# mcgill-cpslab/all-pairs-similarity

Measured on AMD Instinct MI355X. Metric: scored candidate pairs/sec + achieved HBM GB/s, N=1M d=100k nnz=100, 1/2/4/8 GPU, higher is better.
Workload: dtype u16+f32

## Files before the change

all-pairs-similarity_amd/csrc/apss_hip.hip:

```cpp
#include <hip/hip_runtime.h>

#include <algorithm>
#include <cmath>
#include <cstdio>
#include <cstdlib>
#include <cstring>
#include <new>
#include <string>
#include <vector>

#include "../../include/apss.h"
#include "apss_kernels.hpp"
#include "apss_head.hpp"
#include "apss_even.hpp"
#include "apss_topk.hpp"

using namespace apss;

namespace {

thread_local std::string g_create_error;

template <class T>
struct DevBuf {
  T *p = nullptr;
  size_t cap = 0;
};

struct DebugCfg {
  bool build_lds = false;
  bool build_atomic = false;
  bool build_stream = false;
  bool build_runs = false;
  int run_range = 0;
  int run_lanes = 0;
  int run_sub = -1;
  bool build_trace = false;
  bool chunk8 = false;
  bool shard_exact = false;
  bool diag = false;
  bool force_general = false;
  bool exact_accum = false;
  bool big_u5 = false;
  int cx_tile = 0;
  int window = 0;
  int chunks = 0;
  int tiles_per_launch = 0;
  bool no_tail = false;
  bool no_acc8 = false;
  int flat_group = -1;
  int pad_lds = 0;
  bool longpf = false;
  bool even_wide = false;
  bool no_even = false;
  int seg_align = 0;
  bool bank_order = false;
  int fold_w = 0;
  bool no_sym = false;
  int mix = 0;
  bool no_chain = false;
  bool no_append = false;
  bool no_bucket = false;
  int bucket_range = 0;
  int res_cap = 0;
  bool head_bf16 = false;
  int merge = -1;
  bool no_merge_prune = false;
  int merge_u = 0;
  int merge_single = 0;
};

DebugCfg parse_debug_env() {
  DebugCfg d;
  const char *e = getenv("APSS_DEBUG");
  if (!e) return d;
  std::string str(e);
  size_t pos = 0;
  while (pos <= str.size()) {
    const size_t end = std::min(str.find(',', pos), str.size());
    const std::string tok = str.substr(pos, end - pos);
    pos = end + 1;
    const size_t eq = tok.find('=');
    const std::string key = tok.substr(0, eq);
    const int val = eq == std::string::npos ? 1 : atoi(tok.c_str() + eq + 1);
    if (key == "build_lds") d.build_lds = val != 0;
    else if (key == "build_atomic") d.build_atomic = val != 0;
    else if (key == "build_stream") d.build_stream = val != 0;
    else if (key == "build_runs") d.build_runs = val != 0;
    else if (key == "run_range") d.run_range = val;
    else if (key == "run_lanes") d.run_lanes = val;
    else if (key == "run_sub") d.run_sub = val;
    else if (key == "build_trace") d.build_trace = val != 0;
    else if (key == "chunk8") d.chunk8 = val != 0;
    else if (key == "shard_exact") d.shard_exact = val != 0;
    else if (key == "diag") d.diag = val != 0;
    else if (key == "force_general") d.force_general = val != 0;
    else if (key == "exact_accum") d.exact_accum = val != 0;
    else if (key == "big_u5") d.big_u5 = val != 0;
    else if (key == "cx_tile") d.cx_tile = val;
    else if (key == "window") d.window = val;
    else if (key == "chunks") d.chunks = val;
    else if (key == "tiles_per_launch") d.tiles_per_launch = val;
    else if (key == "no_tail") d.no_tail = val != 0;
    else if (key == "no_acc8") d.no_acc8 = val != 0;
    else if (key == "no_even") d.no_even = val != 0;
    else if (key == "even_wide") d.even_wide = val != 0;
    else if (key == "longpf") d.longpf = val != 0;
    else if (key == "pad_lds") d.pad_lds = (int)val;
    else if (key == "flat_group") d.flat_group = (int)val;
    else if (key == "seg_align") d.seg_align = val;
    else if (key == "bank_order") d.bank_order = val != 0;
    else if (key == "fold_w") d.fold_w = val;
    else if (key == "mix") d.mix = val;
    else if (key == "no_sym") d.no_sym = val != 0;
    else if (key == "no_chain") d.no_chain = val != 0;
    else if (key == "no_append") d.no_append = val != 0;
    else if (key == "head_bf16") d.head_bf16 = val != 0;
    else if (key == "res_cap") d.res_cap = val;
    else if (key == "no_bucket") d.no_bucket = val != 0;
    else if (key == "bucket_range") d.bucket_range = val;
    else if (key == "merge") d.merge = (int)val;
    else if (key == "merge_u") d.merge_u = (int)val;
    else if (key == "no_merge_prune") d.no_merge_prune = val != 0;
    else if (key == "merge_single") d.merge_single = (int)val;
    else if (key == "relayout_fail") {}
    else if (!key.empty()) fprintf(stderr, "[apss] unknown APSS_DEBUG token '%s' ignored\n", key.c_str());
  }
  return d;
}

}

struct apss_handle {
  apss_config cfg{};
  DebugCfg dbgcfg;
  int dev = 0;
  hipStream_t own_stream = nullptr;
  hipStream_t stream = nullptr;
  hipEvent_t ev0 = nullptr, ev1 = nullptr;
  std::string err;
  bool sharded = false;
  bool nonneg = true;
  bool q_nonneg = true;
  bool no_acc8 = false;
  uint32_t downgrades = 0;
  int64_t store_max_nnz = 0, q_max_nnz = 0;
  float store_max_norm2 = 0.f, q_max_norm2 = 0.f;
  int64_t store_nonempty = 0;
  int64_t last_batch_nonempty = 0;
  int32_t cb = 16384;
  bool stored_rows = false;

  int64_t n_rows = 0, nnz = 0;
  int64_t idx_rows = 0;
  DevBuf<int64_t> rowptr, ext;
  DevBuf<int32_t> idx;
  DevBuf<uint32_t> erow;
  DevBuf<float> val, sub;
  struct IndexSet {
    int32_t cb = 0;
    int32_t align = 0;
    bool coarse = false;
    int64_t n_tiles = 0, post_used = 0;
    DevBuf<uint2> seg;
    DevBuf<Posting> post;
    DevBuf<uint32_t> post_c;
    DevBuf<int64_t> base, total;
    DevBuf<uint32_t> scan_part;
    DevBuf<uint32_t> maxlen;
    uint32_t max_seg = 0;
    uint32_t long_segs = 0;
    DevBuf<unsigned long long> chunkw;
    double round_chunks = 0.0;
    std::vector<int64_t> h_base;
    double build_ms = 0;
    int64_t built_rows = 0;
  };
  IndexSet ex, cx;
  bool use_coarse = false;
  int64_t n_tiles = 0;
  int64_t ex_built_rows = 0;
  DevBuf<float> tile_min, tile_min_c;
  DevBuf<int64_t> q_rowptr, q_ext;
  DevBuf<int32_t> q_idx;
  DevBuf<float> q_val, q_sub;
  DevBuf<int64_t> s_keep, s_cnt, s_rowdst, s_nnzdst, in_rowptr, in_ext;
  DevBuf<int64_t> scan_tmp;
  DevBuf<int32_t> in_idx;
  DevBuf<float> s_inv, s_sub, in_val;
  DevBuf<double> in_val64;
  DevBuf<unsigned long long> bk_cnt;
  DevBuf<int64_t> bk_base;
  DevBuf<int32_t> bk_idx;
  DevBuf<uint32_t> bk_erow;
  DevBuf<float> bk_val;
  DevBuf<uint32_t> run_cut;
  DevBuf<uint2> run_ent;
  DevBuf<uint2> app_seg;
  DevBuf<char> app_post;
  DevBuf<int32_t> vq_first, vrow_q;
  DevBuf<int64_t> vrow_ptr, vrow_np, vrow_first;
  DevBuf<int32_t> res_q, res_c, fin_q, fin_c;
  DevBuf<float> res_s, fin_s;
  DevBuf<int32_t> res2_q, res2_c;
  DevBuf<float> res2_s, q_prenorm;
  const int32_t *out_q = nullptr, *out_c = nullptr;
  const float *out_s = nullptr;
  int64_t n_res = -1;
  const int64_t *res_q_ext = nullptr;
  const int64_t *last_q_rowptr = nullptr;
  const int32_t *last_q_idx = nullptr;
  const float *last_q_val = nullptr;
  int64_t last_nq = 0;
  DevBuf<unsigned long long> counters, dbg, chain_ctr;
  DevBuf<unsigned int> flagword;
  char *pin = nullptr;
  DevBuf<char> pack;
  const int64_t *up_rowptr = nullptr, *up_ext = nullptr;
  const int32_t *up_idx = nullptr;
  int32_t head_k = 0;
  bool head_fixed = false;
  int32_t head_fold_w = 128;
  int32_t head_exact = 128;
  int32_t head_fold_user = 0;
  bool merge_off = false;
  bool head_longseg = false;
  int32_t head_part = 0, head_parts = 1;
  int64_t head_eval_rows = 0;
  bool head_blocked = false;
  std::vector<int32_t> head_terms;
  DevBuf<int32_t> head_pos;
  struct TailView {
    DevBuf<int64_t> rowptr;
    DevBuf<int32_t> idx;
    DevBuf<float> val;
    DevBuf<uint32_t> erow;
    int64_t rows = 0, nnz = 0, max_nnz = 0, nonempty = 0, last_nonempty = 0;
  };
  TailView tv, qtv;
  DevBuf<int64_t> tv_cnt, tv_off;
  DevBuf<unsigned int> tv_sum;
  DevBuf<uint16_t> W, q_W;
  bool head_i8 = false;
  float head_s = 0.f;
  DevBuf<unsigned int> head_ovf;
  DevBuf<uint32_t> df;
  DevBuf<unsigned long long> dedup_tab, head_ctr;
  DevBuf<int32_t> uq_q, uq_c;
  DevBuf<float> uq_s;
  int64_t head_nonempty = 0, last_batch_head_nonempty = 0;
  double head_sample_frac = 0.0;
  hipEvent_t ev2 = nullptr, ev3 = nullptr;
  int32_t top_k = 0;
  TopkWork topk;
  apss_topk_info tk{};
  apss_stats st{};
  size_t bytes_reserved = 0;
};

namespace {

#define HIPCHK(h, expr)                                                                              \
  do {                                                                                               \
    hipError_t e_ = (expr);                                                                          \
    if (e_ != hipSuccess) {                                                                          \
      (h)->err = std::string(#expr) + ": " + hipGetErrorString(e_);                                  \
      return e_ == hipErrorOutOfMemory ? APSS_E_NOMEM : APSS_E_DEVICE;                               \
    }                                                                                                \
  } while (0)

#define APSS_TRY(expr)          \
  do {                          \
    int32_t rc_ = (expr);       \
    if (rc_ != APSS_OK) return rc_; \
  } while (0)

int32_t fail(apss_handle *h, int32_t rc, const std::string &msg) {
  h->err = msg;
  return rc;
}

template <class T>
int32_t ensure(apss_handle *h, DevBuf<T> &b, size_t n, size_t keep = 0, bool exact = false) {
  if (n <= b.cap && b.p) return APSS_OK;
  size_t ncap = exact ? n : std::max(n, b.cap + b.cap / 2);
  ncap = std::max<size_t>(ncap, 64);
  T *np = nullptr;
  HIPCHK(h, hipMalloc((void **)&np, ncap * sizeof(T)));
  if (keep && b.p) HIPCHK(h, hipMemcpyAsync(np, b.p, keep * sizeof(T), hipMemcpyDeviceToDevice, h->stream));
  if (b.p) {
    HIPCHK(h, hipStreamSynchronize(h->stream));
    HIPCHK(h, hipFree(b.p));
    h->bytes_reserved -= b.cap * sizeof(T);
  }
  b.p = np;
  b.cap = ncap;
  h->bytes_reserved += ncap * sizeof(T);
  return APSS_OK;
}

template <class T>
void release(DevBuf<T> &b) {
  if (b.p) (void)hipFree(b.p);
  b.p = nullptr;
  b.cap = 0;
}

int32_t enter(apss_handle *h) {
  if (!h) return APSS_E_INVALID;
  hipError_t e = hipSetDevice(h->dev);
  if (e != hipSuccess) return fail(h, APSS_E_DEVICE, std::string("hipSetDevice: ") + hipGetErrorString(e));
  return APSS_OK;
}

inline int64_t ceil_div(int64_t a, int64_t b) { return (a + b - 1) / b; }
constexpr size_t kPinBytes = 256 << 10;
constexpr size_t kPinScalars = 1024;

int32_t scan_i64(apss_handle *h, const int64_t *in, int64_t *out, int64_t n) {
  if (n <= 4 * kScanBlock) {
    hipLaunchKernelGGL(k_scan_i64, dim3(1), dim3(1024), 0, h->stream, in, out, n);
    HIPCHK(h, hipGetLastError());
    return APSS_OK;
  }
  const int64_t nb = ceil_div(n, kScanBlock);
  APSS_TRY(ensure(h, h->scan_tmp, (size_t)(2 * nb + 1)));
  int64_t *sums = h->scan_tmp.p, *offs = h->scan_tmp.p + nb;
  hipLaunchKernelGGL(k_scan_sums, dim3((unsigned)nb), dim3(1024), 0, h->stream, in, sums, n);
  hipLaunchKernelGGL(k_scan_i64, dim3(1), dim3(1024), 0, h->stream, (const int64_t *)sums, offs, nb);
  hipLaunchKernelGGL(k_scan_apply, dim3((unsigned)nb), dim3(1024), 0, h->stream, in, (const int64_t *)offs, out, n, nb);
  HIPCHK(h, hipGetLastError());
  return APSS_OK;
}

int32_t head_setup_rendering(apss_handle *h);
int32_t head_fit_scale(apss_handle *h, double norm2, unsigned char *W, int64_t packed_bytes);
inline void head_pack_rendering(const apss_handle *h, HeadPackArgs &p);

int32_t ingest(apss_handle *h, int64_t n, int64_t nnz, const int64_t *d_rowptr, const int32_t *d_idx,
               const float *d_val, const int64_t *d_ext, bool to_store, int64_t *n_out, int64_t *nnz_out) {
  *n_out = 0;
  *nnz_out = 0;
  if (n == 0) return APSS_OK;
  const uint32_t in_flags = h->stored_rows ? h->cfg.flags & ~(APSS_FLAG_VALUE_PRUNE | APSS_FLAG_ADMISSION | APSS_FLAG_NORMALIZE) : h->cfg.flags;
  const bool transform = h->sharded || (in_flags & (APSS_FLAG_VALUE_PRUNE | APSS_FLAG_ADMISSION | APSS_FLAG_NORMALIZE));
  APSS_TRY(ensure(h, h->s_keep, (size_t)n + 1));
  APSS_TRY(ensure(h, h->s_cnt, (size_t)n + 1));
  APSS_TRY(ensure(h, h->s_inv, (size_t)n));
  APSS_TRY(ensure(h, h->s_sub, (size_t)n));
  APSS_TRY(ensure(h, h->flagword, 4));
  HIPCHK(h, hipMemsetAsync(h->flagword.p, 0, 4 * sizeof(unsigned int), h->stream));

  IngestArgs a{};
  a.n = n;
  a.nnz = nnz;
  a.rowptr = d_rowptr;
  a.idx = d_idx;
  a.val = d_val;
  a.dim = h->cfg.dim;
  a.term_lo = h->cfg.term_lo;
  a.term_hi = h->cfg.term_hi;
  a.flags = in_flags;
  a.theta = (float)h->cfg.theta;
  a.index_threshold = (float)h->cfg.index_threshold;
  a.row_keep = h->s_keep.p;
  a.row_cnt = h->s_cnt.p;
  a.row_inv = h->s_inv.p;
  a.row_sub = h->s_sub.p;
  a.flags_out = h->flagword.p;
  const bool shard_head = h->sharded && h->head_k > 0;
  a.head_pos = shard_head ? h->head_pos.p : nullptr;
  const int threads = 256;
  const int64_t blocks = ceil_div(n * kGroup, threads);
  hipLaunchKernelGGL(k_ingest_count<kGroup>, dim3((unsigned)std::min<int64_t>(blocks, 4096)), dim3(threads), 0, h->stream, a);
  HIPCHK(h, hipGetLastError());

  int64_t dst_row0 = to_store ? h->n_rows : 0, dst_nnz0 = to_store ? h->nnz : 0;
  int64_t kept_rows = n, kept_nnz = nnz;
  unsigned int flags_stack[4] = {0, 0, 0, 0};
  unsigned int *flags_host = h->pin ? reinterpret_cast<unsigned int *>(h->pin + kPinBytes) : flags_stack;
  if (transform) {
    APSS_TRY(ensure(h, h->s_rowdst, (size_t)n + 1));
    APSS_TRY(ensure(h, h->s_nnzdst, (size_t)n + 1));
    APSS_TRY(scan_i64(h, (const int64_t *)h->s_keep.p, h->s_rowdst.p, n));
    APSS_TRY(scan_i64(h, (const int64_t *)h->s_cnt.p, h->s_nnzdst.p, n));
    HIPCHK(h, hipGetLastError());
    HIPCHK(h, hipMemcpyAsync(&kept_rows, h->s_rowdst.p + n, sizeof(int64_t), hipMemcpyDeviceToHost, h->stream));
    HIPCHK(h, hipMemcpyAsync(&kept_nnz, h->s_nnzdst.p + n, sizeof(int64_t), hipMemcpyDeviceToHost, h->stream));
  }
  HIPCHK(h, hipMemcpyAsync(flags_host, h->flagword.p, 4 * sizeof(unsigned int), hipMemcpyDeviceToHost, h->stream));
  HIPCHK(h, hipStreamSynchronize(h->stream));
  if (flags_host[0] & 1u)
    return fail(h, APSS_E_INVALID, "malformed vector: indices must be strictly increasing and in [0, dim) "
                                   "(SparseVector.scala:75; vectorDim mismatch is the require of CommonUtils.scala:99)");
  if (flags_host[0] & 2u) return fail(h, APSS_E_INVALID, "non-finite value in a vector");
  if (to_store) h->nonneg = h->nonneg && !(flags_host[0] & 4u);
  else h->q_nonneg = !(flags_host[0] & 4u);
  float norm2;
  std::memcpy(&norm2, &flags_host[2], sizeof(float));
  if (to_store) {
    h->store_max_nnz = std::max<int64_t>(h->store_max_nnz, flags_host[1]);
    h->store_max_norm2 = std::max(h->store_max_norm2, norm2);
    h->store_nonempty += flags_host[3];
    h->last_batch_nonempty = flags_host[3];
  } else {
    h->q_max_nnz = flags_host[1];
    h->q_max_norm2 = norm2;
  }

  DevBuf<int64_t> &o_rowptr = to_store ? h->rowptr : h->q_rowptr;
  DevBuf<int64_t> &o_ext = to_store ? h->ext : h->q_ext;
  DevBuf<int32_t> &o_idx = to_store ? h->idx : h->q_idx;
  DevBuf<float> &o_val = to_store ? h->val : h->q_val;
  DevBuf<float> &o_sub = to_store ? h->sub : h->q_sub;
  APSS_TRY(ensure(h, o_rowptr, (size_t)(dst_row0 + kept_rows + 1), (size_t)(to_store ? dst_row0 + 1 : 0)));
  APSS_TRY(ensure(h, o_ext, (size_t)(dst_row0 + kept_rows), (size_t)dst_row0));
  APSS_TRY(ensure(h, o_idx, (size_t)(dst_nnz0 + kept_nnz), (size_t)dst_nnz0));
  APSS_TRY(ensure(h, o_val, (size_t)(dst_nnz0 + kept_nnz), (size_t)dst_nnz0));
  if (to_store) APSS_TRY(ensure(h, h->erow, (size_t)(dst_nnz0 + kept_nnz), (size_t)dst_nnz0));
  if (h->sharded) APSS_TRY(ensure(h, o_sub, (size_t)(dst_row0 + kept_rows), (size_t)dst_row0));
  if (dst_row0 == 0) HIPCHK(h, hipMemsetAsync(o_rowptr.p, 0, sizeof(int64_t), h->stream));

  IngestWriteArgs w{};
  w.in = a;
  w.dst_row0 = dst_row0;
  w.dst_nnz0 = dst_nnz0;
  w.o_rowptr = o_rowptr.p;
  w.o_idx = o_idx.p;
  w.o_val = o_val.p;
  w.o_ext = o_ext.p;
  w.o_sub = h->sharded ? o_sub.p : nullptr;
  w.o_erow = to_store ? h->erow.p : nullptr;
  w.ext = d_ext;
  if (transform) {
    w.row_dst = h->s_rowdst.p;
    w.nnz_dst = h->s_nnzdst.p;
  } else {
    w.row_dst = nullptr;
    w.nnz_dst = d_rowptr;
  }
  hipLaunchKernelGGL(k_ingest_write, dim3((unsigned)blocks), dim3(threads), 0, h->stream, w);
  HIPCHK(h, hipGetLastError());
  if (shard_head) {
    const int64_t kh = h->head_k;
    DevBuf<uint16_t> &o_W = to_store ? h->W : h->q_W;
    const int64_t rows_end = dst_row0 + kept_rows;
    const int64_t w_pad = to_store ? ceil_div(rows_end, kHeadQBlock) * kHeadQBlock + kHeadCTile : ceil_div(rows_end, kHeadCTile) * kHeadCTile;
    APSS_TRY(ensure(h, o_W, (size_t)(w_pad * kh), (size_t)(ceil_div(dst_row0, kHeadCTile) * kHeadCTile * kh)));
    APSS_TRY(ensure(h, h->head_ctr, 4));
    HIPCHK(h, hipMemsetAsync(h->head_ctr.p, 0, 4 * sizeof(unsigned long long), h->stream));
    if (to_store && dst_row0 == 0) APSS_TRY(head_setup_rendering(h));
    APSS_TRY(head_fit_scale(h, to_store ? (double)h->store_max_norm2 : std::max((double)h->store_max_norm2, (double)h->q_max_norm2),
                            reinterpret_cast<unsigned char *>(h->W.p), ceil_div(to_store ? dst_row0 : h->n_rows, kHeadCTile) * kHeadCTile * kh));
    HeadPackArgs p{};
    head_pack_rendering(h, p);
    p.rowptr = d_rowptr;
    p.idx = d_idx;
    p.val = d_val;
    p.row0 = 0;
    p.row1 = n;
    p.head_pos = h->head_pos.p;
    p.kh = (int32_t)kh;
    p.W = o_W.p;
    p.w_row0 = dst_row0;
    p.w_pad = w_pad;
    p.ratio_t = nullptr;
    p.head_nonempty = reinterpret_cast<unsigned int *>(h->head_ctr.p);
    p.row_inv = (in_flags & APSS_FLAG_NORMALIZE) ? h->s_inv.p : nullptr;
    p.prune_above = (in_flags & APSS_FLAG_VALUE_PRUNE) ? (float)h->cfg.index_threshold : -INFINITY;
    p.fold_from = h->head_exact;
    p.part = h->head_part;
    p.n_parts = h->head_parts;
    hipLaunchKernelGGL(k_head_pack, dim3((unsigned)(ceil_div(w_pad, 8) - dst_row0 / 8)), dim3(512), 0, h->stream, p);
    HIPCHK(h, hipGetLastError());
    if (to_store) {
      unsigned int nz = 0;
      HIPCHK(h, hipMemcpyAsync(&nz, h->head_ctr.p, sizeof(nz), hipMemcpyDeviceToHost, h->stream));
      HIPCHK(h, hipStreamSynchronize(h->stream));
      if (dst_row0 == 0) h->head_nonempty = 0;
      h->head_nonempty += nz;
      h->last_batch_head_nonempty = nz;
    }
  }
  *n_out = kept_rows;
  *nnz_out = kept_nnz;
  return APSS_OK;
}

void fill_build_args(apss_handle *h, apss_handle::IndexSet &ix, BuildArgs &b, bool scaled) {
  b.rowptr = h->head_k ? h->tv.rowptr.p : h->rowptr.p;
  b.idx = h->head_k ? h->tv.idx.p : h->idx.p;
  b.val = h->head_k ? h->tv.val.p : h->val.p;
  b.cb = (int32_t)ix.cb;
  b.dim = h->cfg.dim;
  b.tile_seg = ix.seg.p;
  b.seg_stride = (int64_t)h->cfg.dim;
  b.coarse = ix.coarse ? 1 : 0;
  b.seg_align = ix.align;
  b.erow = h->head_k ? h->tv.erow.p : h->erow.p;
  b.row_scale = scaled && ix.coarse ? h->sub.p : nullptr;
  b.coarse_shift = ix.coarse && ix.cb <= 32768 ? 1 : 0;
  b.coarse_wide = ix.coarse && ix.cb > 65536 ? 1 : 0;
  b.tile_post_base = ix.base.p;
  b.post = ix.post.p;
  b.post_c = ix.post_c.p;
  b.term_lo = h->cfg.term_lo;
  b.term_hi = h->cfg.term_hi;
}

int32_t launch_tile_scan(apss_handle *h, apss_handle::IndexSet &ix, int64_t tile0, int64_t n, uint32_t keep_len, unsigned long long *chunk_w,
                         uint32_t count_long) {
  const int32_t n_blk = (int32_t)ceil_div(h->cfg.dim, kScanBlock);
  APSS_TRY(ensure(h, ix.scan_part, (size_t)(n * n_blk)));
  const dim3 grid((unsigned)(n * n_blk));
  hipLaunchKernelGGL(k_tile_scan_part, grid, dim3(1024), 0, h->stream, (const uint2 *)ix.seg.p, (int64_t)h->cfg.dim, h->cfg.dim, tile0, n_blk,
                     (uint32_t)ix.align, ix.scan_part.p, ix.maxlen.p, chunk_w, count_long);
  hipLaunchKernelGGL(k_tile_scan_place, grid, dim3(1024), 0, h->stream, ix.seg.p, (int64_t)h->cfg.dim, h->cfg.dim, tile0, n_blk, (uint32_t)ix.align,
                     keep_len, (const uint32_t *)ix.scan_part.p, ix.total.p);
  HIPCHK(h, hipGetLastError());
  return APSS_OK;
}

int32_t append_tile(apss_handle *h, apss_handle::IndexSet &ix, int64_t tile, int64_t row0, int64_t row1) {
  const int64_t stride = (int64_t)h->cfg.dim;
  const bool scaled = h->sharded || h->head_k > 0;
  const size_t elt = ix.coarse ? sizeof(uint32_t) : sizeof(Posting);
  const int64_t base = ix.h_base[(size_t)tile], old_total = ix.h_base[(size_t)tile + 1] - base;
  uint2 *sg = ix.seg.p + tile * stride;
  APSS_TRY(ensure(h, h->app_seg, (size_t)stride));
  APSS_TRY(ensure(h, h->app_post, (size_t)std::max<int64_t>(old_total, 1) * elt));
  HIPCHK(h, hipEventRecord(h->ev0, h->stream));
  HIPCHK(h, hipMemcpyAsync(h->app_seg.p, sg, (size_t)stride * sizeof(uint2), hipMemcpyDeviceToDevice, h->stream));
  if (old_total > 0)
    HIPCHK(h, hipMemcpyAsync(h->app_post.p, ix.coarse ? (const void *)(ix.post_c.p + base) : (const void *)(ix.post.p + base),
                             (size_t)old_total * elt, hipMemcpyDeviceToDevice, h->stream));
  BuildArgs b{};
  fill_build_args(h, ix, b, scaled);
  b.row0 = row0;
  b.row1 = row1;
  const int threads = 256;
  const int64_t blocks = ceil_div((row1 - row0) * kWave, threads);
  hipLaunchKernelGGL(k_tile_hist, dim3((unsigned)blocks), dim3(threads), 0, h->stream, b);
  APSS_TRY(launch_tile_scan(h, ix, tile, 1, 0u, nullptr, 0u));
  HIPCHK(h, hipGetLastError());
  int64_t new_total = 0;
  uint32_t seg_stats[2] = {0, 0};
  HIPCHK(h, hipMemcpyAsync(&new_total, ix.total.p + tile, sizeof(int64_t), hipMemcpyDeviceToHost, h->stream));
  HIPCHK(h, hipMemcpyAsync(seg_stats, ix.maxlen.p, sizeof(seg_stats), hipMemcpyDeviceToHost, h->stream));
  HIPCHK(h, hipStreamSynchronize(h->stream));
  ix.max_seg = seg_stats[0];
  ix.h_base[(size_t)tile + 1] = base + new_total;
  ix.post_used = base + new_total;
  if (ix.coarse) APSS_TRY(ensure(h, ix.post_c, (size_t)ix.post_used + 64, (size_t)base));
  else APSS_TRY(ensure(h, ix.post, (size_t)ix.post_used + 64, (size_t)base));
  if (ix.coarse)
    HIPCHK(h, hipMemsetAsync(ix.post_c.p + base, 0, (size_t)(new_total + 64) * sizeof(uint32_t), h->stream));
  HIPCHK(h, hipMemcpyAsync(ix.base.p + tile + 1, ix.h_base.data() + tile + 1, sizeof(int64_t), hipMemcpyHostToDevice, h->stream));
  ShiftArgs sa{};
  sa.seg_old = h->app_seg.p;
  sa.seg_new = sg;
  sa.old_c = ix.coarse ? reinterpret_cast<const uint32_t *>(h->app_post.p) : nullptr;
  sa.old_x = ix.coarse ? nullptr : reinterpret_cast<const Posting *>(h->app_post.p);
  sa.new_c = ix.coarse ? ix.post_c.p + base : nullptr;
  sa.new_x = ix.coarse ? nullptr : ix.post.p + base;
  sa.dim = h->cfg.dim;
  hipLaunchKernelGGL(k_tile_shift, dim3((unsigned)ceil_div(stride * kGroup, 256)), dim3(256), 0, h->stream, sa);
  fill_build_args(h, ix, b, scaled);
  b.row0 = row0;
  b.row1 = row1;
  hipLaunchKernelGGL(k_tile_scatter, dim3((unsigned)blocks), dim3(threads), 0, h->stream, b);
  if (scaled) {
    DevBuf<float> &tmin = ix.coarse ? h->tile_min_c : h->tile_min;
    hipLaunchKernelGGL(k_tile_min_sub, dim3(1), dim3(1024), 0, h->stream, (const float *)h->sub.p, h->idx_rows, (int32_t)ix.cb, tmin.p, tile);
  }
  HIPCHK(h, hipGetLastError());
  HIPCHK(h, hipEventRecord(h->ev1, h->stream));
  HIPCHK(h, hipEventSynchronize(h->ev1));
  float ms = 0.f;
  HIPCHK(h, hipEventElapsedTime(&ms, h->ev0, h->ev1));
  ix.build_ms = ms;
  return APSS_OK;
}

constexpr double kRunMinMeanRow = 20.0;
constexpr int kRunSub = 256;
template <int SCATTER>
void launch_tile_runs(int lanes, dim3 grid, size_t lds, hipStream_t stream, const BuildArgs &b, int64_t tile0, int32_t n_ranges) {
  if (lanes == 4) hipLaunchKernelGGL((k_tile_runs<SCATTER, 4>), grid, dim3(1024), lds, stream, b, tile0, n_ranges);
  else if (lanes == 8) hipLaunchKernelGGL((k_tile_runs<SCATTER, 8>), grid, dim3(1024), lds, stream, b, tile0, n_ranges);
  else if (lanes == 16) hipLaunchKernelGGL((k_tile_runs<SCATTER, 16>), grid, dim3(1024), lds, stream, b, tile0, n_ranges);
  else hipLaunchKernelGGL((k_tile_runs<SCATTER, 32>), grid, dim3(1024), lds, stream, b, tile0, n_ranges);
}

int32_t build_tiles(apss_handle *h, apss_handle::IndexSet &ix, int64_t row0) {
  const int64_t cb = ix.cb;
  int64_t tile0 = row0 / cb;
  const int64_t n_tiles = ceil_div(h->idx_rows, cb);
  const int64_t stride = (int64_t)h->cfg.dim;
  double appended_ms = 0.0;
  if (row0 % cb != 0 && ix.built_rows == row0 && ix.n_tiles == tile0 + 1 && (int64_t)ix.h_base.size() == tile0 + 2 &&
      !h->dbgcfg.no_append && !h->dbgcfg.bank_order) {
    DevBuf<float> &tmin_a = ix.coarse ? h->tile_min_c : h->tile_min;
    if (h->sharded || h->head_k > 0) APSS_TRY(ensure(h, tmin_a, (size_t)n_tiles, (size_t)tile0 + 1));
    APSS_TRY(ensure(h, ix.total, (size_t)n_tiles, (size_t)tile0 + 1));
    APSS_TRY(append_tile(h, ix, tile0, row0, std::min<int64_t>(h->idx_rows, (tile0 + 1) * cb)));
    appended_ms = ix.build_ms;
    ++tile0;
    row0 = tile0 * cb;
    if (h->idx_rows <= row0) {
      ix.built_rows = h->idx_rows;
      return APSS_OK;
    }
  }
  ix.n_tiles = n_tiles;
  ix.built_rows = h->idx_rows;
  if (n_tiles == tile0) return APSS_OK;
  APSS_TRY(ensure(h, ix.seg, (size_t)(n_tiles * stride), (size_t)(tile0 * stride)));
  APSS_TRY(ensure(h, ix.base, (size_t)n_tiles + 1, (size_t)tile0 + 1));
  APSS_TRY(ensure(h, ix.total, (size_t)n_tiles, 0));
  APSS_TRY(ensure(h, ix.maxlen, 2));
  APSS_TRY(ensure(h, ix.chunkw, 1));
  if (tile0 == 0) {
    HIPCHK(h, hipMemsetAsync(ix.maxlen.p, 0, 2 * sizeof(uint32_t), h->stream));
    HIPCHK(h, hipMemsetAsync(ix.chunkw.p, 0, sizeof(unsigned long long), h->stream));
  }
  DevBuf<float> &tmin = ix.coarse ? h->tile_min_c : h->tile_min;
  const bool scaled = h->sharded || h->head_k > 0;
  if (scaled) APSS_TRY(ensure(h, tmin, (size_t)n_tiles, (size_t)tile0));
  if (ix.h_base.empty()) ix.h_base.push_back(0);
  ix.h_base.resize((size_t)tile0 + 1);
  const int64_t r0 = tile0 * cb;
  int32_t n_ranges = (int32_t)ceil_div(h->cfg.dim, kBuildRange);
  const int64_t build_nnz = h->head_k ? h->tv.nnz : h->nnz;
  int32_t bucket_rt = h->dbgcfg.bucket_range > 0 ? h->dbgcfg.bucket_range : 8192;
  while (ceil_div(h->cfg.dim, bucket_rt) > kBucketMaxRanges && bucket_rt < kBuildRange) bucket_rt *= 2;
  const bool bucket_build = n_ranges > kBuildMaxRanges && ceil_div(h->cfg.dim, bucket_rt) <= kBucketMaxRanges && !h->dbgcfg.build_atomic &&
                            !h->dbgcfg.no_bucket && tile0 == 0 && n_tiles * n_ranges >= 48 && build_nnz > 0 && build_nnz <= (1LL << 32) &&
                            n_tiles * (int64_t)kBucketSlices < (1LL << 31);
  if (bucket_build) n_ranges = (int32_t)ceil_div(h->cfg.dim, bucket_rt);
  const bool lds_build = bucket_build || (n_ranges <= kBuildMaxRanges && !h->dbgcfg.build_atomic &&
                                          ((n_tiles - tile0) * n_ranges >= 48 || h->dbgcfg.build_lds));
  if (!lds_build)
    HIPCHK(h, hipMemsetAsync(ix.seg.p + tile0 * stride, 0, (size_t)((n_tiles - tile0) * stride) * sizeof(uint2), h->stream));
  const double mean_row = h->idx_rows > 0 ? (double)build_nnz / (double)h->idx_rows : 0.0;
  int32_t run_rt = h->dbgcfg.run_range > 0 ? std::min(h->dbgcfg.run_range, kBuildRange) : kRunRange;
  const int64_t t_lo = h->cfg.term_lo, t_hi = h->cfg.term_hi;
  const int64_t run_active = std::max<int64_t>(1, ceil_div(t_hi, run_rt) - t_lo / run_rt);
  const double mean_run = mean_row / (double)run_active;
  const bool run_build = lds_build && !bucket_build && !h->dbgcfg.build_stream && std::max<int64_t>(h->store_max_nnz, 1) * cb < (1LL << 31) &&
                         ceil_div(h->cfg.dim, run_rt) <= 64 &&
                         (h->dbgcfg.build_runs || (n_ranges >= 2 && mean_row >= kRunMinMeanRow));
  if (run_build) n_ranges = (int32_t)ceil_div(h->cfg.dim, run_rt);
  BuildArgs b{};
  fill_build_args(h, ix, b, scaled);
  b.row0 = r0;
  b.row1 = h->idx_rows;
  int32_t run_sub = h->dbgcfg.run_sub >= 0 ? h->dbgcfg.run_sub : kRunSub;
  if (run_sub < 64 || run_sub > kPlaceMaxTerms || (run_sub & (run_sub - 1)) || run_rt % run_sub || !ix.coarse || build_nnz > (int64_t)6e8 || build_nnz <= 0)
    run_sub = 0;
  const int32_t n_sub = run_sub ? (int32_t)ceil_div(h->cfg.dim, run_sub) : 0;
  const int64_t n_bk = (n_tiles - tile0) * n_sub;
  const double run_want = run_sub ? mean_run * 0.5 : mean_run;
  int run_lanes = h->dbgcfg.run_lanes;
  if (run_lanes != 4 && run_lanes != 8 && run_lanes != 16 && run_lanes != 32)
    run_lanes = run_want <= 4.0 ? 4 : (run_want <= 8.0 ? 8 : (run_want <= 16.0 ? 16 : 32));
  if (h->dbgcfg.build_trace)
    fprintf(stderr, "[apss] build %s tiles [%lld, %lld): %s, %d ranges of %d terms, %d lanes per row (mean run %.2f)\n", ix.coarse ? "coarse" : "exact",
            (long long)tile0, (long long)n_tiles, bucket_build ? "bucketed" : (run_build ? "runs" : (lds_build ? "stream" : "atomic")), (int)n_ranges,
            run_build ? run_rt : (bucket_build ? bucket_rt : kBuildRange), run_build ? run_lanes : 0, mean_run);
  if (h->dbgcfg.build_trace && run_build) fprintf(stderr, "[apss]   scatter through sub-ranges of %d terms\n", (int)run_sub);
  if (run_build) {
    APSS_TRY(ensure(h, h->run_cut, (size_t)((h->idx_rows - r0) * (n_ranges + 1))));
    b.range_terms = run_rt;
    b.run_cut = h->run_cut.p;
    if (run_sub) {
      APSS_TRY(ensure(h, h->bk_cnt, (size_t)n_bk + 2));
      APSS_TRY(ensure(h, h->bk_base, (size_t)n_bk + 2));
      APSS_TRY(ensure(h, h->run_ent, (size_t)build_nnz));
      int sh = 0;
      while ((1 << sh) < run_sub) ++sh;
      b.sub_shift = sh;
      b.n_sub = n_sub;
      b.sub_cnt = h->bk_cnt.p;
      b.sub_base = h->bk_base.p;
      b.o_ent = h->run_ent.p;
    }
  }
  const int threads = 256;
  const int64_t blocks = ceil_div((h->idx_rows - r0) * kWave, threads);
  HIPCHK(h, hipEventRecord(h->ev0, h->stream));
  int64_t group_tiles = n_tiles;
  BucketArgs bk{};
  if (bucket_build) {
    const int64_t per_tile = std::max<int64_t>(1, build_nnz / n_tiles);
    group_tiles = std::max<int64_t>(1, std::min<int64_t>(n_tiles, (int64_t)6e8 / per_tile));
    std::vector<int64_t> grp_e;
    {
      std::vector<int64_t> at;
      for (int64_t g0 = 0; g0 < n_tiles; g0 += group_tiles) at.push_back(std::min<int64_t>(h->idx_rows, g0 * cb));
      at.push_back(h->idx_rows);
      grp_e.resize(at.size());
      for (size_t i = 0; i < at.size(); ++i)
        HIPCHK(h, hipMemcpyAsync(&grp_e[i], b.rowptr + at[i], sizeof(int64_t), hipMemcpyDeviceToHost, h->stream));
      HIPCHK(h, hipStreamSynchronize(h->stream));
    }
    int64_t max_e = 1;
    for (size_t i = 0; i + 1 < grp_e.size(); ++i) max_e = std::max(max_e, grp_e[i + 1] - grp_e[i]);
    const int64_t nb = group_tiles * n_ranges;
    APSS_TRY(ensure(h, h->bk_cnt, (size_t)(2 * nb + 2)));
    APSS_TRY(ensure(h, h->bk_base, (size_t)nb + 2));
    APSS_TRY(ensure(h, h->bk_idx, (size_t)max_e));
    APSS_TRY(ensure(h, h->bk_erow, (size_t)max_e));
    APSS_TRY(ensure(h, h->bk_val, (size_t)max_e));
    bk.rowptr = b.rowptr;
    bk.idx = b.idx;
    bk.val = b.val;
    bk.erow = b.erow;
    bk.row1 = h->idx_rows;
    bk.cb = (int32_t)cb;
    bk.n_ranges = n_ranges;
    bk.range_terms = bucket_rt;
    bk.bucket_cnt = h->bk_cnt.p;
    bk.bucket_cur = h->bk_cnt.p + nb + 1;
    bk.bucket_base = h->bk_base.p;
    bk.o_idx = h->bk_idx.p;
    bk.o_erow = h->bk_erow.p;
    bk.o_val = h->bk_val.p;
    HIPCHK(h, hipEventRecord(h->ev0, h->stream));
  }
  auto bucket_group = [&](int64_t g0, int64_t gt) -> int32_t {
    const int64_t nbg = gt * n_ranges;
    HIPCHK(h, hipMemsetAsync(h->bk_cnt.p, 0, (size_t)(2 * (group_tiles * n_ranges) + 2) * sizeof(unsigned long long), h->stream));
    bk.tile0 = g0;
    const dim3 bgrid((unsigned)(gt * kBucketSlices));
    hipLaunchKernelGGL(k_bucket_pass<false>, bgrid, dim3(1024), 0, h->stream, bk);
    APSS_TRY(scan_i64(h, reinterpret_cast<const int64_t *>(h->bk_cnt.p), h->bk_base.p, nbg));
    hipLaunchKernelGGL(k_bucket_pass<true>, bgrid, dim3(1024), 0, h->stream, bk);
    HIPCHK(h, hipGetLastError());
    return APSS_OK;
  };
  if (bucket_build) {
    b.idx = h->bk_idx.p;
    b.erow = h->bk_erow.p;
    b.val = h->bk_val.p;
    b.ent_base = h->bk_base.p;
    b.range_terms = bucket_rt;
    for (int64_t g0 = 0; g0 < n_tiles; g0 += group_tiles) {
      const int64_t gt = std::min<int64_t>(group_tiles, n_tiles - g0);
      APSS_TRY(bucket_group(g0, gt));
      hipLaunchKernelGGL(k_tile_hist_lds, dim3((unsigned)(gt * n_ranges)), dim3(1024), 0, h->stream, b, g0, n_ranges);
    }
    HIPCHK(h, hipGetLastError());
  }
  const dim3 lds_grid((unsigned)((n_tiles - tile0) * n_ranges));
  const size_t run_lds = (size_t)run_rt * sizeof(uint32_t);
  if (bucket_build) {}
  else if (run_build) {
    hipLaunchKernelGGL(k_row_cuts, dim3((unsigned)ceil_div((h->idx_rows - r0) * kGroup, threads)), dim3(threads), 0, h->stream, b, n_ranges,
                       h->run_cut.p);
    launch_tile_runs<kRunHist>(run_lanes, lds_grid, run_lds, h->stream, b, tile0, n_ranges);
    if (run_sub) {
      APSS_TRY(scan_i64(h, reinterpret_cast<const int64_t *>(h->bk_cnt.p), h->bk_base.p, n_bk));
      launch_tile_runs<kRunPartition>(run_lanes, lds_grid, run_lds, h->stream, b, tile0, n_ranges);
    }
  } else if (lds_build) hipLaunchKernelGGL(k_tile_hist_lds, lds_grid, dim3(1024), 0, h->stream, b, tile0, n_ranges);
  else hipLaunchKernelGGL(k_tile_hist, dim3((unsigned)blocks), dim3(threads), 0, h->stream, b);
  APSS_TRY(launch_tile_scan(h, ix, tile0, n_tiles - tile0, lds_build ? 1u : 0u, tile0 == 0 ? ix.chunkw.p : nullptr, 1u));
  HIPCHK(h, hipGetLastError());
  std::vector<int64_t> tot((size_t)(n_tiles - tile0));
  HIPCHK(h, hipMemcpyAsync(tot.data(), ix.total.p + tile0, tot.size() * sizeof(int64_t), hipMemcpyDeviceToHost, h->stream));
  uint32_t seg_stats[2] = {0, 0};
  unsigned long long chunk_w = 0;
  HIPCHK(h, hipMemcpyAsync(seg_stats, ix.maxlen.p, sizeof(seg_stats), hipMemcpyDeviceToHost, h->stream));
  HIPCHK(h, hipMemcpyAsync(&chunk_w, ix.chunkw.p, sizeof(chunk_w), hipMemcpyDeviceToHost, h->stream));
  HIPCHK(h, hipStreamSynchronize(h->stream));
  ix.max_seg = seg_stats[0];
  ix.long_segs = seg_stats[1];
  if (tile0 == 0 && h->idx_rows > 0) ix.round_chunks = (double)chunk_w / (double)h->idx_rows;
  for (size_t i = 0; i < tot.size(); ++i) ix.h_base.push_back(ix.h_base.back() + tot[i]);
  HIPCHK(h, hipMemcpyAsync(ix.base.p + tile0, ix.h_base.data() + tile0, (size_t)(n_tiles - tile0 + 1) * sizeof(int64_t),
                           hipMemcpyHostToDevice, h->stream));
  ix.post_used = ix.h_base.back();
  if (ix.coarse) APSS_TRY(ensure(h, ix.post_c, (size_t)ix.post_used + 64, (size_t)ix.h_base[(size_t)tile0]));
  else APSS_TRY(ensure(h, ix.post, (size_t)ix.post_used + 64, (size_t)ix.h_base[(size_t)tile0]));
  if (ix.coarse)
    HIPCHK(h, hipMemsetAsync(ix.post_c.p + ix.h_base[(size_t)tile0], 0,
                             (size_t)(ix.post_used - ix.h_base[(size_t)tile0] + 64) * sizeof(uint32_t), h->stream));
  b.tile_post_base = ix.base.p;
  b.post = ix.post.p;
  b.post_c = ix.post_c.p;
  if (bucket_build) {
    for (int64_t g0 = 0; g0 < n_tiles; g0 += group_tiles) {
      const int64_t gt = std::min<int64_t>(group_tiles, n_tiles - g0);
      if (group_tiles < n_tiles) APSS_TRY(bucket_group(g0, gt));
      hipLaunchKernelGGL(k_tile_scatter_lds, dim3((unsigned)(gt * n_ranges)), dim3(1024), 0, h->stream, b, g0, n_ranges);
    }
  } else if (run_build && run_sub) {
    hipLaunchKernelGGL(k_tile_place_sub, dim3((unsigned)n_bk), dim3(kPlaceBlock), 0, h->stream, b, tile0);
  } else if (run_build) launch_tile_runs<kRunScatter>(run_lanes, lds_grid, run_lds, h->stream, b, tile0, n_ranges);
  else if (lds_build) hipLaunchKernelGGL(k_tile_scatter_lds, lds_grid, dim3(1024), 0, h->stream, b, tile0, n_ranges);
  else hipLaunchKernelGGL(k_tile_scatter, dim3((unsigned)blocks), dim3(threads), 0, h->stream, b);
  if (ix.coarse && ix.cb <= 32768 && h->dbgcfg.bank_order)
    hipLaunchKernelGGL(k_seg_bank_order, dim3((unsigned)ceil_div((n_tiles - tile0) * stride * kWave, 256)), dim3(256), 0, h->stream,
                       (const uint2 *)ix.seg.p, stride, (const int64_t *)ix.base.p, ix.post_c.p, tile0, n_tiles, h->cfg.dim);
  if (scaled)
    hipLaunchKernelGGL(k_tile_min_sub, dim3((unsigned)(n_tiles - tile0)), dim3(1024), 0, h->stream,
                       (const float *)h->sub.p, h->idx_rows, (int32_t)cb, tmin.p, tile0);
  HIPCHK(h, hipGetLastError());
  HIPCHK(h, hipEventRecord(h->ev1, h->stream));
  HIPCHK(h, hipEventSynchronize(h->ev1));
  float ms = 0.f;
  HIPCHK(h, hipEventElapsedTime(&ms, h->ev0, h->ev1));
  ix.build_ms = ms + appended_ms;
  return APSS_OK;
}

int32_t ensure_exact_index(apss_handle *h) {
  if (h->ex_built_rows < h->idx_rows || h->ex.n_tiles == 0) {
    APSS_TRY(build_tiles(h, h->ex, std::min(h->ex_built_rows, h->idx_rows)));
    h->ex_built_rows = h->idx_rows;
    h->st.build_ms += h->ex.build_ms;
  }
  return APSS_OK;
}

double acc8_scale(double bound, double shared, double theta) {
  for (int k = 7; k >= 5; --k) {
    const double S = std::ldexp(1.0, k);
    if (bound * 1.0005 * S < 255.0 - shared && std::floor(theta * S * (1.0 - 1.0 / 2048 - 1e-6)) - 2 >= 12.0) return S;
  }
  return 0.0;
}

constexpr int64_t kTailMaxRows = 1024;
constexpr int64_t kTailMaxBatch = 64;
constexpr int64_t kTailMaxPairs = 1 << 22;
constexpr int32_t kHeadMaxTerms = kHeadBlock * (1 + kHeadMaxFold);
inline int32_t head_width(int32_t n_terms, int32_t fold_w, int32_t exact = kHeadBlock, bool i8 = false) {
  return n_terms <= 64 ? (i8 ? 128 : 64) : (n_terms <= 128 ? 128 : (n_terms <= 256 ? 256 : exact + fold_w));
}
inline int32_t head_column(int32_t i, int32_t fold_w, int32_t exact = kHeadBlock) { return i < exact ? i : exact + (i - exact) % fold_w; }
constexpr int64_t kHeadMinRows = 16384;
constexpr double kHeadSparseRate = 8.0e11;
constexpr double kHeadDenseCost[4] = {1.5e-13, 1.9e-13, 3.1e-13, 3.1e-13};
constexpr double kHeadDenseCostI8[4] = {1.2e-13, 1.2e-13, 1.75e-13, 1.75e-13};
constexpr double kHeadFoldMaxRowTerms = 96.0;
constexpr double kHeadSurvivorCost = 2.5e-9;

inline bool head_allowed(const apss_handle *h) {
  return h->use_coarse && (!h->sharded || h->head_fixed) && (h->cfg.head_terms >= 0 || h->head_fixed) && h->cfg.theta > 0.0 &&
         !h->head_blocked && h->nonneg;
}

inline bool head_wants_i8(const apss_handle *h) {
  return !h->dbgcfg.head_bf16 && !(h->dbgcfg.fold_w == 128 || h->dbgcfg.fold_w == 256);
}
int32_t head_setup_rendering(apss_handle *h) {
  h->head_i8 = h->head_k > 0 && h->head_k <= kHeadBlock && head_wants_i8(h);
  h->head_s = 0.f;
  APSS_TRY(ensure(h, h->head_ovf, 4));
  HIPCHK(h, hipMemsetAsync(h->head_ovf.p, 0, 4 * sizeof(unsigned int), h->stream));
  return APSS_OK;
}
int32_t head_fit_scale(apss_handle *h, double norm2, unsigned char *W, int64_t packed_bytes) {
  if (!h->head_i8) return APSS_OK;
  const double need = 127.0 / (std::sqrt(std::max(norm2, 1e-30)) * 1.0005);
  if (h->head_s > 0.f && need >= (double)h->head_s) return APSS_OK;
  if (h->head_s > 0.f && packed_bytes > 0) {
    const double target = need / 1.25;
    const uint32_t den = 65535u;
    const uint32_t num = (uint32_t)std::min<double>(den, std::ceil(target / (double)h->head_s * den));
    hipLaunchKernelGGL(k_head_rescale, dim3((unsigned)std::min<int64_t>(8192, ceil_div(packed_bytes, 16 * 256))), dim3(256), 0, h->stream, W,
                       packed_bytes / 16 * 16, num, den);
    HIPCHK(h, hipGetLastError());
    h->head_s = (float)target;
  } else {
    h->head_s = (float)need;
  }
  return APSS_OK;
}
inline void head_pack_rendering(const apss_handle *h, HeadPackArgs &p) {
  p.i8_scale = h->head_i8 ? h->head_s : 0.f;
  p.overflow = h->head_ovf.p;
}

int32_t build_tail_view(apss_handle *h, apss_handle::TailView &v, const int64_t *rowptr, const int32_t *idx, const float *val,
                        int64_t row0, int64_t row1, int64_t dst_row0, bool with_erow) {
  const int64_t n = row1 - row0;
  if (dst_row0 == 0) v.rows = v.nnz = v.max_nnz = v.nonempty = 0;
  v.last_nonempty = 0;
  APSS_TRY(ensure(h, v.rowptr, (size_t)(dst_row0 + n + 1), (size_t)(dst_row0 ? dst_row0 + 1 : 0)));
  if (dst_row0 == 0) HIPCHK(h, hipMemsetAsync(v.rowptr.p, 0, sizeof(int64_t), h->stream));
  if (n <= 0) return APSS_OK;
  APSS_TRY(ensure(h, h->tv_cnt, (size_t)n + 1));
  APSS_TRY(ensure(h, h->tv_off, (size_t)n + 1));
  APSS_TRY(ensure(h, h->tv_sum, 2));
  HIPCHK(h, hipMemsetAsync(h->tv_sum.p, 0, 2 * sizeof(unsigned int), h->stream));
  TailViewArgs a{};
  a.rowptr = rowptr;
  a.idx = idx;
  a.val = val;
  a.row0 = row0;
  a.row1 = row1;
  a.head_pos = h->head_pos.p;
  a.cnt = h->tv_cnt.p;
  a.summary = h->tv_sum.p;
  const unsigned blocks = (unsigned)ceil_div(n * kGroup, 256);
  hipLaunchKernelGGL(k_tailv_count, dim3(blocks), dim3(256), 0, h->stream, a);
  HIPCHK(h, hipGetLastError());
  APSS_TRY(scan_i64(h, (const int64_t *)h->tv_cnt.p, h->tv_off.p, n));
  int64_t total = 0;
  unsigned int sum[2] = {0, 0};
  HIPCHK(h, hipMemcpyAsync(&total, h->tv_off.p + n, sizeof(int64_t), hipMemcpyDeviceToHost, h->stream));
  HIPCHK(h, hipMemcpyAsync(sum, h->tv_sum.p, sizeof(sum), hipMemcpyDeviceToHost, h->stream));
  HIPCHK(h, hipStreamSynchronize(h->stream));
  const int64_t nnz0 = v.nnz;
  APSS_TRY(ensure(h, v.idx, (size_t)std::max<int64_t>(nnz0 + total, 1), (size_t)nnz0));
  APSS_TRY(ensure(h, v.val, (size_t)std::max<int64_t>(nnz0 + total, 1), (size_t)nnz0));
  if (with_erow) APSS_TRY(ensure(h, v.erow, (size_t)std::max<int64_t>(nnz0 + total, 1), (size_t)nnz0));
  a.off = h->tv_off.p;
  a.dst_row0 = dst_row0;
  a.dst_nnz0 = nnz0;
  a.o_rowptr = v.rowptr.p;
  a.o_idx = v.idx.p;
  a.o_val = v.val.p;
  a.o_erow = with_erow ? v.erow.p : nullptr;
  hipLaunchKernelGGL(k_tailv_write, dim3(blocks), dim3(256), 0, h->stream, a);
  HIPCHK(h, hipGetLastError());
  v.rows = dst_row0 + n;
  v.nnz = nnz0 + total;
  v.max_nnz = std::max<int64_t>(v.max_nnz, sum[0]);
  v.nonempty += sum[1];
  v.last_nonempty = sum[1];
  return APSS_OK;
}

int32_t head_pack_store(apss_handle *h, int64_t row0) {
  const int64_t kh = h->head_k;
  const int64_t rows_pad = ceil_div(h->idx_rows, kHeadQBlock) * kHeadQBlock + kHeadCTile;
  APSS_TRY(ensure(h, h->W, (size_t)(rows_pad * kh), (size_t)(ceil_div(row0, kHeadCTile) * kHeadCTile * kh)));
  APSS_TRY(ensure(h, h->sub, (size_t)h->idx_rows, (size_t)row0));
  APSS_TRY(ensure(h, h->head_ctr, 4));
  HIPCHK(h, hipMemsetAsync(h->head_ctr.p, 0, 4 * sizeof(unsigned long long), h->stream));
  if (row0 == 0) APSS_TRY(head_setup_rendering(h));
  APSS_TRY(head_fit_scale(h, (double)h->store_max_norm2, reinterpret_cast<unsigned char *>(h->W.p), ceil_div(row0, kHeadCTile) * kHeadCTile * kh));
  {
    HeadPackArgs a{};
    head_pack_rendering(h, a);
    a.rowptr = h->rowptr.p;
    a.idx = h->idx.p;
    a.val = h->val.p;
    a.row0 = row0;
    a.row1 = h->idx_rows;
    a.head_pos = h->head_pos.p;
    a.kh = (int32_t)kh;
    a.W = h->W.p;
    a.w_row0 = row0;
    a.w_pad = rows_pad;
    a.ratio_t = h->sub.p;
    a.head_nonempty = reinterpret_cast<unsigned int *>(h->head_ctr.p);
    a.row_inv = nullptr;
    a.prune_above = -INFINITY;
    a.fold_from = h->head_exact;
    hipLaunchKernelGGL(k_head_pack, dim3((unsigned)(ceil_div(rows_pad, 8) - row0 / 8)), dim3(512), 0, h->stream, a);
  }
  HIPCHK(h, hipGetLastError());
  unsigned int nz = 0;
  HIPCHK(h, hipMemcpyAsync(&nz, h->head_ctr.p, sizeof(nz), hipMemcpyDeviceToHost, h->stream));
  HIPCHK(h, hipStreamSynchronize(h->stream));
  if (row0 == 0) h->head_nonempty = 0;
  h->head_nonempty += nz;
  h->last_batch_head_nonempty = nz;
  return APSS_OK;
}

int32_t run_head(apss_handle *h, const ProbeArgs &a, int64_t nq, int64_t q_slot_base, const uint16_t *Wq, int64_t wq_rows,
                 float thr, double bound, int64_t n_cand);

int32_t head_sample_selectivity(apss_handle *h, double *frac) {
  *frac = 0.0;
  const int64_t kh = h->head_k;
  const int64_t S = std::min<int64_t>(h->idx_rows, 8192), Q = std::min<int64_t>(S, 512);
  const int64_t rows_pad = ceil_div(h->idx_rows, kHeadQBlock) * kHeadQBlock + kHeadCTile;
  APSS_TRY(ensure(h, h->W, (size_t)(rows_pad * kh), 0));
  APSS_TRY(ensure(h, h->sub, (size_t)h->idx_rows, 0));
  APSS_TRY(ensure(h, h->head_ctr, 4));
  APSS_TRY(ensure(h, h->counters, kCtrCount));
  HIPCHK(h, hipMemsetAsync(h->head_ctr.p, 0, 4 * sizeof(unsigned long long), h->stream));
  APSS_TRY(head_setup_rendering(h));
  APSS_TRY(head_fit_scale(h, (double)h->store_max_norm2, nullptr, 0));
  HeadPackArgs p{};
  head_pack_rendering(h, p);
  p.rowptr = h->rowptr.p;
  p.idx = h->idx.p;
  p.val = h->val.p;
  p.row0 = 0;
  p.row1 = S;
  p.head_pos = h->head_pos.p;
  p.kh = (int32_t)kh;
  p.W = h->W.p;
  p.w_row0 = 0;
  p.w_pad = ceil_div(S, kHeadQBlock) * kHeadQBlock;
  p.ratio_t = h->sub.p;
  p.head_nonempty = nullptr;
  p.row_inv = nullptr;
  p.prune_above = -INFINITY;
  p.fold_from = h->head_exact;
  hipLaunchKernelGGL(k_head_pack, dim3((unsigned)ceil_div(p.w_pad, 8)), dim3(512), 0, h->stream, p);
  HIPCHK(h, hipGetLastError());
  constexpr size_t kSampleCap = 1 << 20;
  APSS_TRY(ensure(h, h->res_q, kSampleCap));
  APSS_TRY(ensure(h, h->res_c, kSampleCap));
  APSS_TRY(ensure(h, h->res_s, kSampleCap));
  ProbeArgs a{};
  a.q_ext = h->ext.p;
  a.res_q = h->res_q.p;
  a.res_c = h->res_c.p;
  a.res_s = h->res_s.p;
  a.res_cap = kSampleCap;
  a.counters = h->head_ctr.p + 2;
  const double bound = (double)h->store_max_norm2 * 1.0001 + 1e-6;
  APSS_TRY(run_head(h, a, Q, -1, h->W.p, p.w_pad, (float)(h->cfg.theta - 0.0080 * bound - 1e-5), bound, S));
  unsigned long long c[4];
  HIPCHK(h, hipMemcpyAsync(c, h->head_ctr.p, sizeof(c), hipMemcpyDeviceToHost, h->stream));
  HIPCHK(h, hipStreamSynchronize(h->stream));
  const double pairs = (double)Q * (double)S - (double)Q;
  unsigned long long n_true = 0;
  if (c[2] > 0 && c[2] <= kSampleCap) {
    APSS_TRY(ensure(h, h->fin_q, (size_t)c[2]));
    APSS_TRY(ensure(h, h->fin_c, (size_t)c[2]));
    APSS_TRY(ensure(h, h->fin_s, (size_t)c[2]));
    HIPCHK(h, hipMemsetAsync(h->head_ctr.p, 0, sizeof(unsigned long long), h->stream));
    RescoreArgs r{};
    r.n_pairs = (int64_t)c[2];
    r.q_row = h->res_q.p;
    r.c_slot = h->res_c.p;
    r.q_rowptr = h->rowptr.p;
    r.q_idx = h->idx.p;
    r.q_val = h->val.p;
    r.c_rowptr = h->rowptr.p;
    r.c_idx = h->idx.p;
    r.c_val = h->val.p;
    r.theta = (float)h->cfg.theta;
    r.out_q = h->fin_q.p;
    r.out_c = h->fin_c.p;
    r.out_s = h->fin_s.p;
    r.out_count = h->head_ctr.p;
    hipLaunchKernelGGL(k_rescore, dim3((unsigned)std::max<int64_t>(1, ceil_div(r.n_pairs, (int64_t)kRescorePairs * kRescoreTrips))), dim3(kRescoreBlock), 0, h->stream, r);
    HIPCHK(h, hipGetLastError());
    HIPCHK(h, hipMemcpyAsync(&n_true, h->head_ctr.p, sizeof(n_true), hipMemcpyDeviceToHost, h->stream));
    HIPCHK(h, hipStreamSynchronize(h->stream));
  }
  *frac = pairs > 0 ? (double)(c[2] - std::min(n_true, c[2])) / pairs : 0.0;
  return APSS_OK;
}

int32_t choose_head(apss_handle *h, bool *changed) {
  *changed = false;
  const int64_t n = h->n_rows;
  const int32_t dim = h->cfg.dim;
  h->head_eval_rows = n;
  const int64_t stride = std::max<int64_t>(1, n / 65536);
  const int64_t sampled = ceil_div(n, stride);
  APSS_TRY(ensure(h, h->df, (size_t)dim));
  HIPCHK(h, hipMemsetAsync(h->df.p, 0, (size_t)dim * sizeof(uint32_t), h->stream));
  hipLaunchKernelGGL(k_df_sample, dim3((unsigned)ceil_div(sampled * kWave, 256)), dim3(256), 0, h->stream,
                     (const int64_t *)h->rowptr.p, (const int32_t *)h->idx.p, n, stride, h->df.p);
  HIPCHK(h, hipGetLastError());
  std::vector<uint32_t> df((size_t)dim);
  HIPCHK(h, hipMemcpyAsync(df.data(), h->df.p, (size_t)dim * sizeof(uint32_t), hipMemcpyDeviceToHost, h->stream));
  HIPCHK(h, hipStreamSynchronize(h->stream));
  std::vector<int32_t> order((size_t)dim);
  for (int32_t t = 0; t < dim; ++t) order[(size_t)t] = t;
  const size_t top = (size_t)std::min<int32_t>(dim, kHeadMaxTerms);
  const auto more_frequent = [&](int32_t x, int32_t y) { return df[(size_t)x] != df[(size_t)y] ? df[(size_t)x] > df[(size_t)y] : x < y; };
  bool hopeless = false;
  if (h->cfg.head_terms == 0) {
    double s2_all = 0.0, f_max = 0.0;
    for (int32_t t = 0; t < dim; ++t) {
      const double f = (double)df[(size_t)t] / (double)sampled;
      s2_all += f * f;
      f_max = std::max(f_max, f);
    }
    const double *cost = head_wants_i8(h) ? kHeadDenseCostI8 : kHeadDenseCost;
    const double terms_of[4] = {64.0, 128.0, 256.0, (double)top};
    hopeless = true;
    for (int ki = 0; ki < 4; ++ki)
      if (std::min(s2_all, terms_of[ki] * f_max * f_max) / kHeadSparseRate >= 1.5 * 0.5 * cost[ki]) hopeless = false;
  }
  if (!hopeless) {
    std::nth_element(order.begin(), order.begin() + (ptrdiff_t)top - 1, order.end(), more_frequent);
    std::sort(order.begin(), order.begin() + (ptrdiff_t)top, more_frequent);
  }
  int32_t k = 0;
  double best_gain = 0.0;
  double gain256 = 0.0;
  if (h->cfg.head_terms > 0) {
    k = std::min(h->cfg.head_terms <= 256 ? head_width(h->cfg.head_terms, 0) : h->cfg.head_terms, kHeadMaxTerms);
  } else if (n >= kHeadMinRows && !hopeless) {
    double best = 0.0, s2 = 0.0;
    size_t i = 0;
    int ki = 0;
    double m_fold = 0.0;
    for (int32_t kk : {64, 128, 256, 512, 1024, 2048, 4096, 8192, 16384, 32768}) {
      if (kk > kHeadMaxTerms || (size_t)kk > top + 255) break;
      for (; i < std::min<size_t>(top, (size_t)kk); ++i) {
        const double f = (double)df[(size_t)order[i]] / (double)sampled;
        s2 += f * f;
        if (i >= (size_t)h->head_exact) m_fold += f;
      }
      if (m_fold > kHeadFoldMaxRowTerms) break;
      const double save = s2 / kHeadSparseRate, cost = 0.5 * (head_wants_i8(h) ? kHeadDenseCostI8 : kHeadDenseCost)[std::min(ki++, 3)];
      if (save >= 1.5 * cost && kk == kHeadBlock) gain256 = save - cost;
      if (save >= 1.5 * cost && save - cost > best) {
        best = save - cost;
        k = kk;
      }
    }
    best_gain = best;
  }
  if (std::min(k, kHeadBlock) > dim) k = 0;
  std::vector<int32_t> terms;
  for (size_t i = 0; i < std::min<size_t>(top, (size_t)k); ++i)
    if (df[(size_t)order[i]] > 0) terms.push_back(order[i]);
  const int32_t old_k = h->head_k;
  const std::vector<int32_t> old_terms = h->head_terms;
  auto upload_columns = [&]() -> int32_t {
    std::vector<int32_t> pos((size_t)dim, -1);
    for (size_t i = 0; i < h->head_terms.size(); ++i) pos[(size_t)h->head_terms[i]] = head_column((int32_t)i, h->head_fold_w, h->head_exact);
    APSS_TRY(ensure(h, h->head_pos, (size_t)dim));
    HIPCHK(h, hipMemcpyAsync(h->head_pos.p, pos.data(), (size_t)dim * sizeof(int32_t), hipMemcpyHostToDevice, h->stream));
    HIPCHK(h, hipStreamSynchronize(h->stream));
    return APSS_OK;
  };
  for (;;) {
    k = terms.empty() ? 0 : head_width((int32_t)terms.size(), h->head_fold_w, h->head_exact, head_wants_i8(h));
    const bool differs = k != old_k || terms != old_terms;
    h->head_k = k;
    h->head_terms = terms;
    if (k && differs) APSS_TRY(upload_columns());
    if (!(k && differs && h->cfg.head_terms == 0)) break;
    double frac = 0.0;
    APSS_TRY(head_sample_selectivity(h, &frac));
    h->head_sample_frac = frac;
    if (frac * kHeadSurvivorCost <= 0.5 * best_gain) break;
    if (terms.size() > (size_t)kHeadBlock && gain256 > 0.0) {
      terms.resize((size_t)kHeadBlock);
      best_gain = gain256;
      continue;
    }
    h->head_k = 0;
    h->head_terms.clear();
    break;
  }
  *changed = h->head_k != old_k || h->head_terms != old_terms;
  return APSS_OK;
}

int32_t build_index(apss_handle *h, int64_t row0) {
  h->st.build_ms = 0;
  row0 = std::min(row0, h->idx_rows);
  h->idx_rows = h->n_rows;
  if (head_allowed(h)) {
    if (!h->head_fixed && h->n_rows >= std::max<int64_t>(h->cfg.head_terms > 0 ? 1 : kHeadMinRows, 2 * h->head_eval_rows)) {
      bool changed = false;
      APSS_TRY(choose_head(h, &changed));
      if (changed) {
        row0 = 0;
        h->cx.n_tiles = 0;
        h->ex_built_rows = 0;
      }
    }
    if (h->head_k) {
      h->cx.cb = std::min(h->cx.cb, 65536);
      if (!h->sharded) APSS_TRY(head_pack_store(h, row0));
      const int64_t tv0 = row0 == h->tv.rows ? row0 : 0;
      APSS_TRY(build_tail_view(h, h->tv, h->rowptr.p, h->idx.p, h->val.p, tv0, h->idx_rows, tv0, true));
    }
  } else if (h->head_k && h->sharded) {
    return fail(h, APSS_E_UNSUPPORTED, "a term shard with a dense-head block needs non-negative weights (apss_set_head_terms)");
  } else if (h->head_k) {
    h->downgrades |= APSS_DOWNGRADE_HEAD;
    h->head_k = 0;
    h->head_terms.clear();
    row0 = 0;
    h->cx.n_tiles = 0;
    h->ex_built_rows = 0;
  }
  if (h->use_coarse) {
    if (h->cx.n_tiles == 0 && h->cfg.tile_rows == 0 && !h->dbgcfg.cx_tile && h->idx_rows > 0) {
      const double seg32 = 32768.0 * ((double)h->nnz / (double)h->n_rows) / (double)h->cfg.dim;
      h->cx.cb = seg32 < 16.0 && !h->sharded && !h->head_k ? 65536 : 32768;
      if (h->cx.cb == 65536 && seg32 < 8.0 && h->nonneg && !h->dbgcfg.no_acc8 && !h->no_acc8 && h->store_max_nnz <= 512 &&
          acc8_scale((double)h->store_max_norm2 * 1.0001 + 1e-6, (double)h->store_max_nnz, h->cfg.theta) > 0)
        h->cx.cb = 131072;
      if ((h->sharded || h->head_k) && !(h->head_k && h->head_longseg) && !h->dbgcfg.no_acc8 && !h->no_acc8 &&
          acc8_scale((double)h->store_max_norm2 * 1.0001 + 1e-6, (double)h->store_max_nnz, h->cfg.theta) > 0)
        h->cx.cb = 65536;
    }
    APSS_TRY(build_tiles(h, h->cx, row0));
    h->st.build_ms += h->cx.build_ms;
    if (h->head_k && h->cfg.tile_rows == 0 && !h->dbgcfg.cx_tile) {
      if (h->cx.cb > 32768 && h->cx.max_seg > (uint32_t)kLongLenW) {
        h->head_longseg = true;
        h->cx.cb = 32768;
        h->cx.n_tiles = 0;
        APSS_TRY(build_tiles(h, h->cx, 0));
        h->st.build_ms += h->cx.build_ms;
      } else if (h->cx.cb <= 32768 && h->head_longseg && row0 == 0 && 2 * h->cx.max_seg <= (uint32_t)kLongLenW) {
        h->head_longseg = false;
      }
    }
    h->ex_built_rows = std::min(h->ex_built_rows, row0 / h->ex.cb * h->ex.cb);
  } else {
    h->ex_built_rows = std::min(h->ex_built_rows, row0);
    APSS_TRY(ensure_exact_index(h));
  }
  h->n_tiles = ceil_div(h->idx_rows, h->ex.cb);
  return APSS_OK;
}

template <int MODE, bool FX, int BLOCK = kProbeBlock>
int32_t launch_probe(apss_handle *h, const ProbeArgs &a, size_t lds) {
  auto kern = k_probe<MODE, BLOCK, FX>;
  HIPCHK(h, hipFuncSetAttribute(reinterpret_cast<const void *>(kern), hipFuncAttributeMaxDynamicSharedMemorySize, (int)lds));
  hipLaunchKernelGGL(kern, dim3((unsigned)((int64_t)a.n_tiles * a.n_chunks)), dim3(BLOCK), lds, h->stream, a);
  HIPCHK(h, hipGetLastError());
  return APSS_OK;
}
inline int gen_block(int mode, int cb) { return mode == 2 && cb <= 8192 ? 512 : kProbeBlock; }

#define APSS_CX_VARIANTS(X)                          \
  X(512, 5, false, 16, false, false, false, false)   \
  X(512, 4, false, 16, false, false, false, false)   \
  X(512, 3, false, 16, false, false, false, false)   \
  X(512, 2, false, 16, false, false, false, false)   \
  X(512, 5, true, 16, false, false, false, false)    \
  X(512, 4, true, 16, false, false, false, false)    \
  X(512, 3, true, 16, false, false, false, false)    \
  X(512, 2, true, 16, false, false, false, false)    \
  X(512, 5, true, 16, false, false, false, true)     \
  X(512, 4, true, 16, false, false, false, true)     \
  X(512, 3, true, 16, false, false, false, true)     \
  X(512, 2, true, 16, false, false, false, true)     \
  X(512, 5, false, 16, false, false, false, true)    \
  X(512, 4, false, 16, false, false, false, true)    \
  X(512, 3, false, 16, false, false, false, true)    \
  X(512, 2, false, 16, false, false, false, true)    \
  X(512, 5, true, 16, false, false, true, false)     \
  X(512, 5, false, 16, false, false, true, false)    \
  X(512, 5, true, 16, true, false, true, false)      \
  X(512, 4, false, 8, false, false, false, false)    \
  X(512, 5, false, 16, true, false, false, false)    \
  X(512, 5, false, 16, false, true, false, false)    \
  X(512, 5, true, 16, false, true, false, false)     \
  X(512, 5, false, 16, true, true, false, false)     \
  X(1024, 5, false, 16, false, false, false, false)  \
  X(1024, 3, false, 16, false, false, false, false)  \
  X(1024, 5, false, 16, true, false, false, false)   \
  X(1024, 3, false, 16, true, false, false, false)   \
  X(1024, 5, false, 16, false, true, false, false)   \
  X(1024, 3, false, 16, false, true, false, false)   \
  X(1024, 5, false, 16, false, false, false, true)   \
  X(1024, 3, false, 16, false, false, false, true)

struct CxVariant {
  int block, u;
  bool shard;
  int chunk;
  bool vrows, sgn;
  bool longpf;
  bool acc8;
  bool even;
  bool merge;
};

#define APSS_EVEN_VARIANTS(X)          \
  X(512, 7, false, false, false)       \
  X(512, 6, false, false, false)       \
  X(512, 5, false, false, false)       \
  X(512, 4, false, false, false)       \
  X(512, 3, false, false, false)       \
  X(512, 2, false, false, false)       \
  X(512, 7, true, false, false)        \
  X(512, 6, true, false, false)        \
  X(512, 5, true, false, false)        \
  X(512, 4, true, false, false)        \
  X(512, 3, true, false, false)        \
  X(512, 2, true, false, false)        \
  X(512, 7, true, false, true)         \
  X(512, 6, true, false, true)         \
  X(512, 5, true, false, true)         \
  X(512, 4, true, false, true)         \
  X(512, 3, true, false, true)         \
  X(512, 2, true, false, true)         \
  X(512, 4, false, false, true)        \
  X(512, 3, false, false, true)        \
  X(512, 2, false, false, true)        \
  X(1024, 7, false, false, false)      \
  X(1024, 6, false, false, false)      \
  X(1024, 5, false, false, false)      \
  X(1024, 3, false, false, false)      \
  X(1024, 7, false, false, true)       \
  X(1024, 6, false, false, true)       \
  X(1024, 5, false, false, true)       \
  X(1024, 3, false, false, true)
#define APSS_EVEN_MERGE_VARIANTS(X) \
  X(7, false) X(6, false) X(5, false) X(4, false) X(3, false) X(2, false) \
  X(7, true) X(6, true) X(5, true) X(4, true) X(3, true) X(2, true)

bool cx_variant_exists(const CxVariant &v) {
  if (v.even && v.merge) {
#define X(U, A8) \
    if (v.block == 512 && v.u == U && v.shard && !v.sgn && v.acc8 == A8) return v.chunk == 16 && !v.vrows && !v.longpf;
    APSS_EVEN_MERGE_VARIANTS(X)
#undef X
    return false;
  }
  if (v.even) {
#define X(B, U, SH, SG, A8) \
    if (v.block == B && v.u == U && v.shard == SH && v.sgn == SG && v.acc8 == A8) return v.chunk == 16 && !v.vrows && !v.longpf;
    APSS_EVEN_VARIANTS(X)
#undef X
    return false;
  }
#define X(B, U, SH, CH, VR, SG, LP, A8)                                                                                 \
  if (v.block == B && v.u == U && v.shard == SH && v.chunk == CH && v.vrows == VR && v.sgn == SG && v.longpf == LP &&   \
      v.acc8 == A8)                                                                                                     \
    return true;
  APSS_CX_VARIANTS(X)
#undef X
  return false;
}

int32_t launch_cx(apss_handle *h, const CxVariant &v, const ProbeArgs &a) {
  const dim3 grid((unsigned)((int64_t)a.n_tiles * a.n_chunks));
  if (v.even && v.merge) {
#define X(U, A8)                                                                                                           \
    if (v.block == 512 && v.u == U && v.acc8 == A8) {                                                                      \
      hipLaunchKernelGGL((k_probe_even_merged<U, A8>), grid, dim3(512), (size_t)h->dbgcfg.pad_lds, h->stream, a);           \
      HIPCHK(h, hipGetLastError());                                                                                        \
      return APSS_OK;                                                                                                      \
    }
    APSS_EVEN_MERGE_VARIANTS(X)
#undef X
    return fail(h, APSS_E_UNSUPPORTED, "no filter kernel for this combination of options");
  }
  if (v.even) {
#define X(B, U, SH, SG, A8)                                                                                                \
    if (v.block == B && v.u == U && v.shard == SH && v.sgn == SG && v.acc8 == A8) {                                        \
      hipLaunchKernelGGL((k_probe_even<B, U, (B <= 512 ? 128 : 256), SH, SG, A8>), grid, dim3(B),                          \
                         (size_t)h->dbgcfg.pad_lds, h->stream, a);                                                                                 \
      HIPCHK(h, hipGetLastError());                                                                                        \
      return APSS_OK;                                                                                                      \
    }
    APSS_EVEN_VARIANTS(X)
#undef X
    return fail(h, APSS_E_UNSUPPORTED, "no filter kernel for this combination of options");
  }
#define X(B, U, SH, CH, VR, SG, LP, A8)                                                                                    \
  if (v.block == B && v.u == U && v.shard == SH && v.chunk == CH && v.vrows == VR && v.sgn == SG && v.longpf == LP &&      \
      v.acc8 == A8) {                                                                                                      \
    hipLaunchKernelGGL((k_probe_coarse<B, U, (B <= 512 ? 128 : 256), (B <= 512 ? 512 : 1024), SH, CH, VR, SG, LP, A8>), grid, dim3(B), \
                       0, h->stream, a);                                                                                   \
    HIPCHK(h, hipGetLastError());                                                                                          \
    return APSS_OK;                                                                                                        \
  }
  APSS_CX_VARIANTS(X)
#undef X
  return fail(h, APSS_E_UNSUPPORTED, "no filter kernel for this combination of options");
}

int32_t run_head(apss_handle *h, const ProbeArgs &a, int64_t nq, int64_t q_slot_base, const uint16_t *Wq, int64_t wq_rows,
                 float thr, double bound, int64_t n_cand) {
  const bool i8 = h->head_i8;
  const double s2 = (double)h->head_s * (double)h->head_s;
  const int32_t thr_i = i8 ? (int32_t)std::max(1.0, std::floor(s2 * (h->cfg.theta - 2e-5 * (1.0 + bound)))) : 0;
  const float inv_s2 = i8 ? (float)(1.0 / s2) : 0.f;
  const int kt = h->head_k;
  const int kh = std::min(kt, kHeadBlock);
  const int n_blocks = kt > kHeadBlock ? 2 : 1;
  const int fold_w = kt - kHeadBlock;
  if (nq <= 2 * kGemvQ) {
    HeadGemvArgs g{};
    g.Wq = Wq;
    g.Wc = h->W.p;
    g.n_rows = n_cand;
    g.q_slot_base = q_slot_base;
    g.nq = (int32_t)nq;
    g.kh = kh;
    g.kt = kt;
    g.part = h->head_part;
    g.n_parts = h->head_parts;
    g.q_ext = a.q_ext;
    g.c_ext = h->ext.p;
    g.thr = i8 ? (float)thr_i : thr;
    g.i8 = i8 ? 1 : 0;
    g.inv_s2 = inv_s2;
    g.res_q = a.res_q;
    g.res_c = a.res_c;
    g.res_s = a.res_s;
    g.res_cap = a.res_cap;
    g.counters = a.counters;
    g.head_pairs = h->head_ctr.p + 1;
    const int64_t blocks = std::min<int64_t>(2048, std::max<int64_t>(1, ceil_div(n_cand, 256 * (int64_t)h->head_parts)));
    for (int b = 0; b < n_blocks; ++b) {
      g.chunk0 = b * (kHeadBlock / 8);
      g.kh = b ? fold_w : kh;
      g.head_pairs = h->head_ctr.p + (b == 0 ? 1 : 3);
      hipLaunchKernelGGL(k_head_gemv, dim3((unsigned)blocks), dim3(256), 0, h->stream, g);
    }
    HIPCHK(h, hipGetLastError());
    h->st.head_flops = 2.0 * kt * (double)nq * (double)n_cand / (double)h->head_parts;
    return APSS_OK;
  }
  HeadGemmArgs g{};
  g.Wq = Wq;
  g.Wc = h->W.p;
  g.wq_rows = wq_rows;
  g.n_rows = n_cand;
  g.q_slot_base = q_slot_base;
  g.nq = (int32_t)nq;
  const int64_t qs0 = q_slot_base >= 0 ? q_slot_base : 0;
  g.qblock0 = qs0 / kHeadQBlock * kHeadQBlock;
  g.n_qblocks = (int32_t)(ceil_div(qs0 + nq, kHeadQBlock) - qs0 / kHeadQBlock);
  const int64_t ct = head_tile_rows(kh);
  g.n_ctiles = (int32_t)ceil_div(n_cand, ct);
  g.part = h->head_part;
  g.n_parts = h->head_parts;
  const int64_t my_ctiles = std::max<int64_t>(1, g.n_ctiles / g.n_parts);
  int64_t panels = 8;
  while (panels * g.n_qblocks < 2048 && my_ctiles / (2 * panels) >= 32) panels *= 2;
  panels = std::max<int64_t>(1, std::min<int64_t>(panels, my_ctiles));
  g.n_panels = (int32_t)panels;
  g.q_ext = a.q_ext;
  g.c_ext = h->ext.p;
  g.thr = thr;
  g.thr_i = thr_i;
  g.inv_s2 = inv_s2;
  g.res_q = a.res_q;
  g.res_c = a.res_c;
  g.res_s = a.res_s;
  g.res_cap = a.res_cap;
  g.counters = a.counters;
  g.head_pairs = h->head_ctr.p + 1;
  g.kt = kt;
  const int64_t all_qblocks = g.n_qblocks, first_qblock0 = g.qblock0;
  const int64_t per_launch = std::max<int64_t>(1, (int64_t)(4e12 / ((double)kHeadQBlock * (double)ct * (double)my_ctiles)));
  for (int b = 0; b < n_blocks; ++b) {
    g.chunk0 = b * (kHeadBlock / 8);
    for (int64_t q0 = 0; q0 < all_qblocks; q0 += per_launch) {
      g.n_qblocks = (int32_t)std::min<int64_t>(per_launch, all_qblocks - q0);
      g.qblock0 = first_qblock0 + q0 * kHeadQBlock;
      const dim3 grid((unsigned)((int64_t)g.n_qblocks * g.n_panels));
      if (i8 && kh == 128) hipLaunchKernelGGL((k_head_gemm<128, true, 3, 8, true>), grid, dim3(512), 0, h->stream, g);
      else if (i8) hipLaunchKernelGGL((k_head_gemm<256, true, 3, 8, true>), grid, dim3(512), 0, h->stream, g);
      else if (b > 0 && fold_w == 128) hipLaunchKernelGGL((k_head_gemm<128, false, 3>), grid, dim3(512), 0, h->stream, g);
      else if (b > 0) hipLaunchKernelGGL((k_head_gemm<256, false, 3>), grid, dim3(512), 0, h->stream, g);
      else if (kh == 64) hipLaunchKernelGGL((k_head_gemm<64, true, 2>), grid, dim3(512), 0, h->stream, g);
      else if (kh == 128) hipLaunchKernelGGL((k_head_gemm<128, true, 2>), grid, dim3(512), 0, h->stream, g);
      else hipLaunchKernelGGL((k_head_gemm<256, true, 3>), grid, dim3(512), 0, h->stream, g);
    }
  }
  g.n_qblocks = (int32_t)all_qblocks;
  g.qblock0 = first_qblock0;
  HIPCHK(h, hipGetLastError());
  double tiles = 0;
  for (int64_t b = 0; b < g.n_qblocks; ++b) {
    const int64_t hi = q_slot_base >= 0 ? std::min<int64_t>(g.n_ctiles, (g.qblock0 + (b + 1) * kHeadQBlock) / ct) : g.n_ctiles;
    tiles += hi > g.part ? (double)ceil_div(hi - g.part, g.n_parts) : 0.0;
  }
  h->st.head_flops = 2.0 * kt * tiles * (double)ct * (double)kHeadQBlock;
  return APSS_OK;
}

struct FilterFacts {
  bool acc8;
  bool shard_rule;
  bool sgn;
  bool hybrid;
  int64_t s_max_nnz, s_nnz_end;
  int64_t nq, idx_nnz;
  int max_merge_log2;
};

int32_t plan_filter(apss_handle *h, const FilterFacts &f, CxVariant &cxv, ProbeArgs &a) {
  const DebugCfg &dbg = h->dbgcfg;
  cxv.acc8 = f.acc8;
  cxv.block = h->cx.cb > 65536 || (h->cx.cb > 32768 && !cxv.acc8) ? 1024 : 512;
  cxv.shard = f.shard_rule;
  cxv.chunk = dbg.chunk8 ? 8 : 16;
  cxv.vrows = f.s_max_nnz > 512;
  cxv.sgn = f.sgn;
  const double nw = cxv.block / kWave;
  const double seg = (double)h->cx.cb * ((double)f.idx_nnz / (double)h->n_rows) / (double)h->cfg.dim;
  double q_terms = (double)f.s_nnz_end / (double)f.nq;
  const double t_hi = f.shard_rule ? q_terms + 3.0 * std::sqrt(q_terms) : q_terms;
  const double wave_chunks = std::ceil(t_hi / nw - 1e-9) * std::max(1.0, seg / 16.0 + (f.shard_rule ? 1.0 : 0.5));
  int u = (int)std::ceil(wave_chunks * (f.shard_rule ? 1.0 : 1.05) / 8.0);
  if (cxv.block == 1024) u = (q_terms / nw) * std::max(1.0, seg / 16.0 + 0.5) <= 17.0 && !dbg.big_u5 ? 3 : 5;
  else u = std::max(2, std::min(5, u));
// ... 564 lines not shown
        sp.c_sub = h->sub.p;
        sp.theta = (float)theta;
        sp.out_q = h->res2_q.p;
        sp.out_c = h->res2_c.p;
        sp.out_s = h->res2_s.p;
        sp.counter = h->counters.p + kCtrResults;
        sp.over = h->counters.p + kCtrOver;
        const int64_t grid_pairs = std::min<int64_t>((int64_t)a.res_cap, nq / 4 + 4096);
        hipLaunchKernelGGL(k_shard_prune, dim3((unsigned)std::min<int64_t>(2048, ceil_div(grid_pairs, kPrunePairs * 4))), dim3(kPruneBlock), 0, h->stream, sp);
        HIPCHK(h, hipGetLastError());
        std::swap(h->res_q, h->res2_q);
        std::swap(h->res_c, h->res2_c);
        std::swap(h->res_s, h->res2_s);
        a.res_q = h->res_q.p;
        a.res_c = h->res_c.p;
        a.res_s = h->res_s.p;
      }
    }
    if (tri) {
      HIPCHK(h, hipMemcpyAsync(h->counters.p + kCtrSnap, h->counters.p + kCtrResults, sizeof(unsigned long long), hipMemcpyDeviceToDevice, h->stream));
      hipLaunchKernelGGL(k_mirror_survivors, dim3(1024), dim3(256), 0, h->stream, a.res_q, a.res_c, a.res_s,
                         (const unsigned long long *)(h->counters.p + kCtrSnap), (uint64_t)a.res_cap, (int32_t)a.cb, h->counters.p + kCtrResults);
      HIPCHK(h, hipGetLastError());
    }
    HIPCHK(h, hipEventRecord(h->ev1, h->stream));
    unsigned long long cc_stack[kCtrCount] = {0, 0, 0, 0, 0, 0, 0, 0}, c_stack[kCtrCount];
    unsigned long long *cc = h->pin ? reinterpret_cast<unsigned long long *>(h->pin + kPinBytes + 64) : cc_stack;
    unsigned long long *c = h->pin ? reinterpret_cast<unsigned long long *>(h->pin + kPinBytes + 128) : c_stack;
    for (int k = 0; k < kCtrCount; ++k) cc[k] = 0;
    if (chain) {
      HIPCHK(h, hipMemsetAsync(h->chain_ctr.p, 0, kCtrCount * sizeof(unsigned long long), h->stream));
      RescoreArgs r{};
      r.n_pairs = (int64_t)a.res_cap;
      r.n_pairs_dev = h->counters.p + kCtrResults;
      r.q_row = h->res_q.p;
      r.c_slot = h->res_c.p;
      r.q_rowptr = q_rowptr;
      r.q_idx = q_idx;
      r.q_val = q_val;
      r.c_rowptr = h->rowptr.p;
      r.c_idx = h->idx.p;
      r.c_val = h->val.p;
      r.theta = (float)theta;
      r.out_q = h->fin_q.p;
      r.out_c = h->fin_c.p;
      r.out_s = h->fin_s.p;
      r.out_count = h->chain_ctr.p + kCtrResults;
      const int64_t grid_pairs = std::min<int64_t>((int64_t)a.res_cap, 64 * nq + 4096);
      hipLaunchKernelGGL(k_rescore, dim3((unsigned)std::max<int64_t>(1, ceil_div(grid_pairs, (int64_t)kRescorePairs * kRescoreTrips))), dim3(kRescoreBlock), 0, h->stream, r);
      if (tail_n > 0) {
        TailArgs t{};
        t.nq = nq;
        t.n_tail = tail_n;
        t.q_rowptr = q_rowptr;
        t.q_idx = q_idx;
        t.q_val = q_val;
        t.q_ext = q_ext;
        t.c_rowptr = h->rowptr.p;
        t.c_idx = h->idx.p;
        t.c_val = h->val.p;
        t.c_ext = h->ext.p;
        t.tail0 = h->idx_rows;
        t.theta = (float)theta;
        t.out_q = h->fin_q.p;
        t.out_c = h->fin_c.p;
        t.out_s = h->fin_s.p;
        t.out_base = 0;
        t.counters = h->chain_ctr.p;
        hipLaunchKernelGGL(k_tail_score, dim3((unsigned)ceil_div(chain_tail_pairs * kGroup, 256)), dim3(256), 0, h->stream, t);
      }
      HIPCHK(h, hipGetLastError());
      HIPCHK(h, hipMemcpyAsync(cc, h->chain_ctr.p, kCtrCount * sizeof(unsigned long long), hipMemcpyDeviceToHost, h->stream));
    }
    unsigned long long sparse_results = 0, head_c[4] = {0, 0, 0, 0};
    if (hybrid) {
      HIPCHK(h, hipMemcpyAsync(&sparse_results, h->counters.p + kCtrResults, sizeof(sparse_results), hipMemcpyDeviceToHost, h->stream));
      HIPCHK(h, hipMemsetAsync(h->head_ctr.p, 0, 4 * sizeof(unsigned long long), h->stream));
      HIPCHK(h, hipEventRecord(h->ev2, h->stream));
      const bool stored = q_slot_base >= 0;
      APSS_TRY(run_head(h, a, nq, q_slot_base, stored ? h->W.p : h->q_W.p, stored ? (int64_t)(h->W.cap / h->head_k) : ceil_div(nq, kHeadCTile) * kHeadCTile, head_thr, bound, h->idx_rows));
      HIPCHK(h, hipEventRecord(h->ev3, h->stream));
      HIPCHK(h, hipMemcpyAsync(head_c, h->head_ctr.p, sizeof(head_c), hipMemcpyDeviceToHost, h->stream));
    }
    HIPCHK(h, hipMemcpyAsync(c, h->counters.p, kCtrCount * sizeof(unsigned long long), hipMemcpyDeviceToHost, h->stream));
    HIPCHK(h, hipStreamSynchronize(h->stream));
    float ms = 0.f;
    HIPCHK(h, hipEventElapsedTime(&ms, h->ev0, h->ev1));
    h->st.probe_ms += ms;
    h->st.probe_launches += n_launches;
    h->st.thin_launches += thin_launches;
    h->st.posting_visits = (int64_t)c[kCtrVisits];
    h->st.device_posting_visits = (int64_t)(tri ? c[kCtrDevVisits] : c[kCtrVisits]);
    h->st.symmetric = tri ? 1u : 0u;
    h->st.candidate_pairs = (int64_t)c[kCtrCands];
    if ((wave_path || coarse_path) && q_slot_base >= 0)
      h->st.candidate_pairs -= h->head_k > 0 ? ((q_slot_base == 0 && nq == h->n_rows) ? h->tv.nonempty : h->tv.last_nonempty)
                                             : ((q_slot_base == 0 && nq == h->n_rows) ? h->store_nonempty : h->last_batch_nonempty);
    if (hybrid) {
      HIPCHK(h, hipEventElapsedTime(&ms, h->ev2, h->ev3));
      h->st.head_ms += ms;
      int64_t self = 0;
      if (q_slot_base >= 0) self = (q_slot_base == 0 && nq == h->n_rows) ? h->head_nonempty : h->last_batch_head_nonempty;
      h->st.head_pairs = (int64_t)head_c[1] - self;
      h->st.head_survivors = (int64_t)(c[kCtrResults] - sparse_results);
      h->st.candidate_pairs = std::max(h->st.candidate_pairs, h->st.head_pairs);
    }
    h->st.result_pairs = (int64_t)c[kCtrResults];
    if (a.merge_log2 > 0 && (int64_t)c[kCtrPre] > (2 * nq + 100000) * (h->sharded && !dbg.no_merge_prune ? (1LL << a.merge_log2) : 1LL))
      h->merge_off = true;
    if (cxv.acc8 && (int64_t)c[kCtrResults] > std::max<int64_t>(64 * nq, 4000000)) {
      h->cx.cb = shard_rule ? 32768 : 65536;
      h->cx.n_tiles = 0;
      h->no_acc8 = true;
      h->downgrades |= APSS_DOWNGRADE_ACC8;
      APSS_TRY(build_index(h, 0));
      return probe_inner(h, nq, q_rowptr, q_idx, q_val, q_ext, q_slot_first, q_max_nnz, q_max_norm2, q_nnz_end, n_results);
    }
    if (std::max(c[kCtrResults], c[kCtrOver]) > a.res_cap) {
      const size_t asked = (size_t)std::max(c[kCtrResults], c[kCtrOver]);
      size_t need = asked + asked / 8 + 1024;
      if (tri) {
        const size_t snap = (size_t)c[kCtrSnap];
        const size_t head_part = hybrid && c[kCtrResults] > sparse_results ? (size_t)(c[kCtrResults] - sparse_results) : 0;
        need = std::max(need, 2 * snap + head_part + (2 * snap + head_part) / 8 + 1024);
      }
      APSS_TRY(ensure(h, h->res_q, need, 0, true));
      APSS_TRY(ensure(h, h->res_c, need, 0, true));
      APSS_TRY(ensure(h, h->res_s, need, 0, true));
      continue;
    }
    if (chain) {
      h->st.filter_survivors = (int64_t)c[kCtrResults];
      h->n_res = (int64_t)cc[kCtrResults];
      h->st.posting_visits += (int64_t)cc[kCtrVisits];
      h->st.device_posting_visits += (int64_t)cc[kCtrVisits];
      h->st.candidate_pairs += (int64_t)cc[kCtrCands];
      h->st.result_pairs = h->n_res;
      h->out_q = h->fin_q.p;
      h->out_c = h->fin_c.p;
      h->out_s = h->fin_s.p;
      if (n_results) *n_results = h->n_res;
      return APSS_OK;
    }
    h->n_res = (int64_t)c[kCtrResults];
    h->out_q = h->res_q.p;
    h->out_c = h->res_c.p;
    h->out_s = h->res_s.p;
    if (coarse_path && h->sharded) h->st.filter_survivors = h->n_res;
    if (coarse_path && !h->sharded) APSS_TRY(exact_pass(h, hybrid, theta, nq, q_rowptr, q_idx, q_val, q_ext, tail_n));
    if (n_results) *n_results = h->n_res;
    return APSS_OK;
  }
  return fail(h, APSS_E_STATE, "result buffer kept overflowing");
}

int32_t probe(apss_handle *h, int64_t nq, const int64_t *q_rowptr, const int32_t *q_idx, const float *q_val,
              const int64_t *q_ext, int64_t q_slot_first, int64_t q_max_nnz, float q_max_norm2,
              int64_t q_nnz_end, int64_t *n_results) {
  h->tk = apss_topk_info{};
  APSS_TRY(probe_inner(h, nq, q_rowptr, q_idx, q_val, q_ext, q_slot_first, q_max_nnz, q_max_norm2, q_nnz_end, n_results));
  h->tk.pairs_over_theta = h->tk.kept = h->n_res;
  if (h->top_k <= 0 || h->sharded) return APSS_OK;
  const size_t before = h->topk.bytes;
  const hipError_t e = topk_run(h->topk, h->stream, h->out_q, h->out_c, h->out_s, h->n_res, nq, h->ext.p, h->n_rows, h->top_k, &h->tk);
  h->bytes_reserved += h->topk.bytes - before;
  if (e != hipSuccess) {
    h->n_res = -1;
    h->err = std::string("per-query top-k: ") + hipGetErrorString(e);
    return e == hipErrorOutOfMemory ? APSS_E_NOMEM : APSS_E_DEVICE;
  }
  if (h->n_res > 0) {
    h->out_q = h->topk.out_q;
    h->out_c = h->topk.out_c;
    h->out_s = h->topk.out_s;
    h->n_res = h->tk.kept;
  }
  h->st.result_pairs = h->n_res;
  if (n_results) *n_results = h->n_res;
  return APSS_OK;
}

int32_t validate_host_csr(apss_handle *h, int64_t n, const int64_t *rowptr, const int32_t *indices,
                          const double *values, const int64_t *ext_ids) {
  if (n < 0) return fail(h, APSS_E_INVALID, "negative row count");
  if (n == 0) return APSS_OK;
  if (!rowptr || !ext_ids) return fail(h, APSS_E_INVALID, "null rowptr / ext_ids");
  if (rowptr[0] != 0) return fail(h, APSS_E_INVALID, "rowptr[0] must be 0");
  for (int64_t i = 0; i < n; ++i)
    if (rowptr[i + 1] < rowptr[i]) return fail(h, APSS_E_INVALID, "rowptr must be non-decreasing");
  if (rowptr[n] > 0 && (!indices || !values)) return fail(h, APSS_E_INVALID, "null indices / values");
  return APSS_OK;
}

__global__ void k_narrow_f64(const double *in, float *out, int64_t n) {
  for (int64_t i = (int64_t)blockIdx.x * blockDim.x + threadIdx.x; i < n; i += (int64_t)gridDim.x * blockDim.x) out[i] = (float)in[i];
}

int32_t upload(apss_handle *h, int64_t n, const int64_t *rowptr, const int32_t *indices, const double *values,
               const int64_t *ext_ids) {
  const int64_t nnz = n ? rowptr[n] : 0;
  APSS_TRY(ensure(h, h->in_val, (size_t)std::max<int64_t>(nnz, 1)));
  const size_t off_ext = (size_t)(n + 1) * sizeof(int64_t), off_val = off_ext + (size_t)n * sizeof(int64_t);
  const size_t off_idx = off_val + (size_t)nnz * sizeof(double), bytes = off_idx + (size_t)nnz * sizeof(int32_t);
  if (n > 0 && h->pin && bytes <= kPinBytes) {
    APSS_TRY(ensure(h, h->pack, kPinBytes));
    std::memcpy(h->pin, rowptr, off_ext);
    std::memcpy(h->pin + off_ext, ext_ids, (size_t)n * sizeof(int64_t));
    if (nnz) {
      std::memcpy(h->pin + off_val, values, (size_t)nnz * sizeof(double));
      std::memcpy(h->pin + off_idx, indices, (size_t)nnz * sizeof(int32_t));
    }
    HIPCHK(h, hipMemcpyAsync(h->pack.p, h->pin, bytes, hipMemcpyHostToDevice, h->stream));
    h->up_rowptr = reinterpret_cast<const int64_t *>(h->pack.p);
    h->up_ext = reinterpret_cast<const int64_t *>(h->pack.p + off_ext);
    h->up_idx = reinterpret_cast<const int32_t *>(h->pack.p + off_idx);
    if (nnz) {
      hipLaunchKernelGGL(k_narrow_f64, dim3((unsigned)std::min<int64_t>(2048, ceil_div(nnz, 256))), dim3(256), 0, h->stream,
                         reinterpret_cast<const double *>(h->pack.p + off_val), h->in_val.p, nnz);
      HIPCHK(h, hipGetLastError());
    }
    return APSS_OK;
  }
  APSS_TRY(ensure(h, h->in_rowptr, (size_t)n + 1));
  APSS_TRY(ensure(h, h->in_ext, (size_t)std::max<int64_t>(n, 1)));
  APSS_TRY(ensure(h, h->in_idx, (size_t)std::max<int64_t>(nnz, 1)));
  APSS_TRY(ensure(h, h->in_val64, (size_t)std::max<int64_t>(nnz, 1)));
  h->up_rowptr = h->in_rowptr.p;
  h->up_ext = h->in_ext.p;
  h->up_idx = h->in_idx.p;
  if (n) {
    HIPCHK(h, hipMemcpyAsync(h->in_rowptr.p, rowptr, (size_t)(n + 1) * sizeof(int64_t), hipMemcpyHostToDevice, h->stream));
    HIPCHK(h, hipMemcpyAsync(h->in_ext.p, ext_ids, (size_t)n * sizeof(int64_t), hipMemcpyHostToDevice, h->stream));
  }
  if (nnz) {
    HIPCHK(h, hipMemcpyAsync(h->in_idx.p, indices, (size_t)nnz * sizeof(int32_t), hipMemcpyHostToDevice, h->stream));
    HIPCHK(h, hipMemcpyAsync(h->in_val64.p, values, (size_t)nnz * sizeof(double), hipMemcpyHostToDevice, h->stream));
    hipLaunchKernelGGL(k_narrow_f64, dim3(2048), dim3(256), 0, h->stream, (const double *)h->in_val64.p, h->in_val.p, nnz);
    HIPCHK(h, hipGetLastError());
  }
  HIPCHK(h, hipStreamSynchronize(h->stream));
  return APSS_OK;
}

int32_t insert_dev_impl(apss_handle *h, int64_t n, int64_t nnz, const int64_t *d_rowptr, const int32_t *d_idx,
                        const float *d_val, const int64_t *d_ext, int64_t *first_new_row) {
  *first_new_row = h->n_rows;
  if (n == 0) return APSS_OK;
  h->n_res = -1;
  h->res_q_ext = nullptr;
  h->last_q_rowptr = nullptr;
  h->last_q_idx = nullptr;
  h->last_q_val = nullptr;
  h->last_nq = 0;
  if (h->n_rows + n > 0x7fffffffLL) return fail(h, APSS_E_INVALID, "more than 2^31 - 1 vectors in one handle");
  int64_t kept_rows = 0, kept_nnz = 0;
  const bool was_nonneg = h->nonneg;
  APSS_TRY(ingest(h, n, nnz, d_rowptr, d_idx, d_val, d_ext, true, &kept_rows, &kept_nnz));
  if (h->sharded && h->head_k && !h->nonneg) {
    h->nonneg = was_nonneg;
    return fail(h, APSS_E_UNSUPPORTED, "a term shard with a dense-head block needs non-negative weights (apss_set_head_terms)");
  }
  const int64_t row0 = h->n_rows;
  h->n_rows += kept_rows;
  h->nnz += kept_nnz;
  const bool tail_ok = h->use_coarse && !h->sharded && h->idx_rows > 0 && !h->dbgcfg.no_tail;
  if (tail_ok && kept_rows <= kTailMaxBatch && h->n_rows - h->idx_rows <= kTailMaxRows) {
    h->st.build_ms = 0;
    return APSS_OK;
  }
  APSS_TRY(build_index(h, row0));
  return APSS_OK;
}

int32_t pack_query_head(apss_handle *h, const int64_t *rowptr, const int32_t *idx, const float *val, int64_t nq) {
  const int64_t q_pad = ceil_div(nq, kHeadCTile) * kHeadCTile;
  APSS_TRY(ensure(h, h->q_W, (size_t)(q_pad * h->head_k)));
  APSS_TRY(ensure(h, h->q_sub, (size_t)nq));
  APSS_TRY(head_fit_scale(h, std::max((double)h->store_max_norm2, (double)h->q_max_norm2), reinterpret_cast<unsigned char *>(h->W.p),
                          ceil_div(h->idx_rows, kHeadCTile) * kHeadCTile * (int64_t)h->head_k));
  HeadPackArgs a{};
  head_pack_rendering(h, a);
  a.rowptr = rowptr;
  a.idx = idx;
  a.val = val;
  a.row0 = 0;
  a.row1 = nq;
  a.head_pos = h->head_pos.p;
  a.kh = h->head_k;
  a.W = h->q_W.p;
  a.w_row0 = 0;
  a.w_pad = q_pad;
  a.ratio_t = h->q_sub.p;
  a.head_nonempty = nullptr;
  a.row_inv = nullptr;
  a.prune_above = -INFINITY;
  a.fold_from = h->head_exact;
  hipLaunchKernelGGL(k_head_pack, dim3((unsigned)ceil_div(q_pad, 8)), dim3(512), 0, h->stream, a);
  HIPCHK(h, hipGetLastError());
  return APSS_OK;
}

int32_t query_dev_impl(apss_handle *h, int64_t n, int64_t nnz, const int64_t *d_rowptr, const int32_t *d_idx,
                       const float *d_val, const int64_t *d_ext, int64_t *n_results) {
  int64_t kept_rows = 0, kept_nnz = 0;
  APSS_TRY(ingest(h, n, nnz, d_rowptr, d_idx, d_val, d_ext, false, &kept_rows, &kept_nnz));
  if (h->head_k && !h->sharded && kept_rows > 0) APSS_TRY(pack_query_head(h, h->q_rowptr.p, h->q_idx.p, h->q_val.p, kept_rows));
  return probe(h, kept_rows, h->q_rowptr.p, h->q_idx.p, h->q_val.p, h->q_ext.p, -1, h->q_max_nnz, h->q_max_norm2, kept_nnz,
               n_results);
}

}

extern "C" {

int32_t apss_create(const apss_config *cfg, apss_handle **out) {
  if (!cfg || !out) {
    g_create_error = "null argument";
    return APSS_E_INVALID;
  }
  *out = nullptr;
  if (cfg->struct_size != (int32_t)sizeof(apss_config)) {
    g_create_error = "apss_config.struct_size mismatch";
    return APSS_E_INVALID;
  }
  if (cfg->dim <= 0 || !std::isfinite(cfg->theta)) {
    g_create_error = "dim must be > 0 and theta finite";
    return APSS_E_INVALID;
  }
  apss_handle *h = new (std::nothrow) apss_handle();
  if (!h) return APSS_E_NOMEM;
  h->cfg = *cfg;
  h->dbgcfg = parse_debug_env();
  if (h->cfg.term_hi == 0 && h->cfg.term_lo == 0) h->cfg.term_hi = cfg->dim;
  if (h->cfg.term_lo < 0 || h->cfg.term_hi > cfg->dim || h->cfg.term_lo >= h->cfg.term_hi) {
    g_create_error = "bad term range";
    delete h;
    return APSS_E_INVALID;
  }
  h->sharded = !(h->cfg.term_lo == 0 && h->cfg.term_hi == cfg->dim);
  h->use_coarse = !(cfg->flags & (APSS_FLAG_EXACT_ACCUM | APSS_FLAG_FORCE_GENERAL | APSS_FLAG_FORCE_SCAN)) &&
                  (!h->sharded || !h->dbgcfg.shard_exact);
  h->cb = cfg->tile_rows ? cfg->tile_rows : (cfg->theta > 0.0 ? 16384 : 8192);
  h->ex.cb = h->cb;
  h->ex.align = kSegAlign;
  h->cx.cb = std::min(2 * h->cb, 32768);
  if (h->dbgcfg.cx_tile) h->cx.cb = h->dbgcfg.cx_tile;
  h->no_acc8 = h->dbgcfg.no_acc8;
  if (h->dbgcfg.fold_w == 128 || h->dbgcfg.fold_w == 256) {
    h->head_exact = 256;
    h->head_fold_w = h->dbgcfg.fold_w;
  } else if (h->dbgcfg.mix >= 32 && h->dbgcfg.mix <= 224 && h->dbgcfg.mix % 32 == 0) {
    h->head_exact = h->dbgcfg.mix;
    h->head_fold_w = 256 - h->dbgcfg.mix;
  }
  h->cx.align = h->dbgcfg.seg_align == 16 ? 16 : kSegAlignC;
  h->cx.coarse = true;
  if (h->cb < 64 || h->cb > 32768 || (h->cb % 64)) {
    g_create_error = "tile_rows must be a multiple of 64 in [64, 32768]";
    delete h;
    return APSS_E_INVALID;
  }
  if (h->sharded && !(cfg->theta > 0.0)) {
    g_create_error = "term-range shards need theta > 0 (candidate test p_g >= theta*|q_g|*|c_g|)";
    delete h;
    return APSS_E_UNSUPPORTED;
  }
  h->dev = cfg->device_id;
  int ndev = 0;
  hipError_t e = hipGetDeviceCount(&ndev);
  if (e != hipSuccess || ndev <= 0 || h->dev < 0 || h->dev >= ndev) {
    g_create_error = std::string("no usable HIP device (there is no CPU fallback): ") +
                     (e != hipSuccess ? hipGetErrorString(e) : "device ordinal out of range");
    delete h;
    return APSS_E_DEVICE;
  }
  if ((e = hipSetDevice(h->dev)) != hipSuccess || (e = hipStreamCreateWithFlags(&h->own_stream, hipStreamDefault)) != hipSuccess ||
      (e = hipEventCreate(&h->ev0)) != hipSuccess || (e = hipEventCreate(&h->ev1)) != hipSuccess ||
      (e = hipEventCreate(&h->ev2)) != hipSuccess || (e = hipEventCreate(&h->ev3)) != hipSuccess) {
    g_create_error = std::string("HIP init failed: ") + hipGetErrorString(e);
    delete h;
    return APSS_E_DEVICE;
  }
  h->stream = h->own_stream;
  if (hipHostMalloc((void **)&h->pin, kPinBytes + kPinScalars, hipHostMallocDefault) != hipSuccess) h->pin = nullptr;
  if (cfg->capacity_rows > 0) {
    if (ensure(h, h->rowptr, (size_t)cfg->capacity_rows + 1, 0, true) != APSS_OK ||
        ensure(h, h->ext, (size_t)cfg->capacity_rows, 0, true) != APSS_OK) {
      g_create_error = h->err;
      apss_destroy(h);
      return APSS_E_NOMEM;
    }
  }
  if (cfg->capacity_nnz > 0) {
    if (ensure(h, h->idx, (size_t)cfg->capacity_nnz, 0, true) != APSS_OK ||
        ensure(h, h->erow, (size_t)cfg->capacity_nnz, 0, true) != APSS_OK ||
        ensure(h, h->val, (size_t)cfg->capacity_nnz, 0, true) != APSS_OK ||
        (h->use_coarse ? ensure(h, h->cx.post_c, (size_t)cfg->capacity_nnz * 2 + 64, 0, true)
                       : ensure(h, h->ex.post, (size_t)cfg->capacity_nnz + (size_t)cfg->capacity_nnz / 2 + 64, 0, true)) != APSS_OK) {
      g_create_error = h->err;
      apss_destroy(h);
      return APSS_E_NOMEM;
    }
  }
  *out = h;
  return APSS_OK;
}

void apss_destroy(apss_handle *h) {
  if (!h) return;
  (void)hipSetDevice(h->dev);
  if (h->own_stream) (void)hipStreamSynchronize(h->own_stream);
  release(h->rowptr); release(h->ext); release(h->idx); release(h->erow); release(h->val); release(h->sub);
  for (apss_handle::IndexSet *s : {&h->ex, &h->cx}) { release(s->seg); release(s->post); release(s->post_c); release(s->base); release(s->total); release(s->maxlen); release(s->chunkw); release(s->scan_part); }
  release(h->tile_min); release(h->tile_min_c); release(h->fin_q); release(h->fin_c); release(h->fin_s);
  release(h->q_rowptr); release(h->q_ext); release(h->q_idx); release(h->q_val); release(h->q_sub);
  release(h->s_keep); release(h->s_cnt); release(h->s_rowdst); release(h->s_nnzdst); release(h->scan_tmp);
  release(h->in_rowptr); release(h->in_ext); release(h->in_idx); release(h->s_inv); release(h->s_sub); release(h->in_val); release(h->in_val64); release(h->vq_first); release(h->vrow_q); release(h->vrow_ptr); release(h->vrow_np); release(h->vrow_first);
  release(h->res_q); release(h->res_c); release(h->res_s); release(h->res2_q); release(h->res2_c); release(h->res2_s); release(h->q_prenorm); release(h->counters); release(h->flagword); release(h->dbg);
  release(h->head_pos); release(h->W);
  for (apss_handle::TailView *v : {&h->tv, &h->qtv}) { release(v->rowptr); release(v->idx); release(v->val); release(v->erow); }
  release(h->tv_cnt); release(h->tv_off); release(h->tv_sum); release(h->q_W); release(h->df); release(h->dedup_tab);
  release(h->head_ctr); release(h->uq_q); release(h->uq_c); release(h->uq_s); release(h->pack); release(h->chain_ctr); release(h->app_seg); release(h->app_post); release(h->bk_cnt); release(h->bk_base); release(h->bk_idx); release(h->bk_erow); release(h->bk_val); release(h->run_cut); release(h->run_ent);
  topk_release(h->topk);
  if (h->pin) (void)hipHostFree(h->pin);
  if (h->ev0) (void)hipEventDestroy(h->ev0);
  if (h->ev1) (void)hipEventDestroy(h->ev1);
  if (h->ev2) (void)hipEventDestroy(h->ev2);
  if (h->ev3) (void)hipEventDestroy(h->ev3);
  if (h->own_stream) (void)hipStreamDestroy(h->own_stream);
  delete h;
}

const char *apss_last_error(const apss_handle *h) { return h ? h->err.c_str() : g_create_error.c_str(); }

int32_t apss_set_stream(apss_handle *h, void *hip_stream, int32_t use_own) {
  APSS_TRY(enter(h));
  HIPCHK(h, hipStreamSynchronize(h->stream));
  h->stream = use_own ? h->own_stream : (hipStream_t)hip_stream;
  return APSS_OK;
}

int32_t apss_insert(apss_handle *h, int64_t n, const int64_t *rowptr, const int32_t *indices, const double *values,
                    const int64_t *ext_ids) {
  APSS_TRY(enter(h));
  APSS_TRY(validate_host_csr(h, n, rowptr, indices, values, ext_ids));
  if (n == 0) return APSS_OK;
  APSS_TRY(upload(h, n, rowptr, indices, values, ext_ids));
  int64_t first = 0;
  return insert_dev_impl(h, n, rowptr[n], h->up_rowptr, h->up_idx, h->in_val.p, h->up_ext, &first);
}

int32_t apss_query(apss_handle *h, int64_t n, const int64_t *rowptr, const int32_t *indices, const double *values,
                   const int64_t *ext_ids, int64_t *n_results) {
  APSS_TRY(enter(h));
  APSS_TRY(validate_host_csr(h, n, rowptr, indices, values, ext_ids));
  APSS_TRY(upload(h, n, rowptr, indices, values, ext_ids));
  return query_dev_impl(h, n, n ? rowptr[n] : 0, h->up_rowptr, h->up_idx, h->in_val.p, h->up_ext, n_results);
}

int32_t apss_insert_and_query(apss_handle *h, int64_t n, const int64_t *rowptr, const int32_t *indices,
                              const double *values, const int64_t *ext_ids, int64_t *n_results) {
  APSS_TRY(enter(h));
  APSS_TRY(validate_host_csr(h, n, rowptr, indices, values, ext_ids));
  APSS_TRY(upload(h, n, rowptr, indices, values, ext_ids));
  return apss_insert_and_query_dev(h, n, n ? rowptr[n] : 0, h->up_rowptr, h->up_idx, h->in_val.p, h->up_ext, n_results);
}

int32_t apss_self_join(apss_handle *h, int64_t *n_results) {
  APSS_TRY(enter(h));
  if (h->idx_rows < h->n_rows) APSS_TRY(build_index(h, h->idx_rows));
  return probe(h, h->n_rows, h->rowptr.p, h->idx.p, h->val.p, h->ext.p, 0, h->store_max_nnz, h->store_max_norm2, h->nnz, n_results);
}

int32_t apss_result_count(const apss_handle *h, int64_t *n_results) {
  if (!h || !n_results) return APSS_E_INVALID;
  if (h->n_res < 0) return APSS_E_STATE;
  *n_results = h->n_res;
  return APSS_OK;
}

__global__ void k_gather_ids(const int32_t *res_q, const int32_t *res_c, const int64_t *q_ext, const int64_t *c_ext,
                             int64_t n, int64_t *out_q, int64_t *out_c) {
  const int64_t i = (int64_t)blockIdx.x * blockDim.x + threadIdx.x;
  if (i < n) {
    out_q[i] = q_ext[res_q[i]];
    out_c[i] = c_ext[res_c[i]];
  }
}

int32_t apss_fetch_results(apss_handle *h, int64_t offset, int64_t count, int64_t *out_q, int64_t *out_c,
                           float *out_score) {
  APSS_TRY(enter(h));
  if (h->n_res < 0) return fail(h, APSS_E_STATE, "no query has run on this handle");
  if (offset < 0 || count < 0 || offset + count > h->n_res) return fail(h, APSS_E_INVALID, "fetch range out of bounds");
  if (count == 0) return APSS_OK;
  if (!out_q || !out_c || !out_score) return fail(h, APSS_E_INVALID, "null output buffer");
  if (h->pin && (size_t)count * 20 <= kPinBytes) {
    APSS_TRY(ensure(h, h->pack, kPinBytes));
    int64_t *pq = reinterpret_cast<int64_t *>(h->pack.p), *pc = pq + count;
    float *ps = reinterpret_cast<float *>(pc + count);
    hipLaunchKernelGGL(k_gather_ids, dim3((unsigned)ceil_div(count, 256)), dim3(256), 0, h->stream, h->out_q + offset, h->out_c + offset,
                       h->res_q_ext, (const int64_t *)h->ext.p, count, pq, pc);
    HIPCHK(h, hipGetLastError());
    HIPCHK(h, hipMemcpyAsync(ps, h->out_s + offset, (size_t)count * sizeof(float), hipMemcpyDeviceToDevice, h->stream));
    HIPCHK(h, hipMemcpyAsync(h->pin, h->pack.p, (size_t)count * 20, hipMemcpyDeviceToHost, h->stream));
    HIPCHK(h, hipStreamSynchronize(h->stream));
    std::memcpy(out_q, h->pin, (size_t)count * sizeof(int64_t));
    std::memcpy(out_c, h->pin + (size_t)count * sizeof(int64_t), (size_t)count * sizeof(int64_t));
    std::memcpy(out_score, h->pin + (size_t)count * 2 * sizeof(int64_t), (size_t)count * sizeof(float));
    return APSS_OK;
  }
  APSS_TRY(ensure(h, h->s_rowdst, (size_t)count));
  APSS_TRY(ensure(h, h->s_nnzdst, (size_t)count));
  hipLaunchKernelGGL(k_gather_ids, dim3((unsigned)ceil_div(count, 256)), dim3(256), 0, h->stream,
                     h->out_q + offset, h->out_c + offset, h->res_q_ext,
                     (const int64_t *)h->ext.p, count, h->s_rowdst.p, h->s_nnzdst.p);
  HIPCHK(h, hipGetLastError());
  HIPCHK(h, hipMemcpyAsync(out_q, h->s_rowdst.p, (size_t)count * sizeof(int64_t), hipMemcpyDeviceToHost, h->stream));
  HIPCHK(h, hipMemcpyAsync(out_c, h->s_nnzdst.p, (size_t)count * sizeof(int64_t), hipMemcpyDeviceToHost, h->stream));
  HIPCHK(h, hipMemcpyAsync(out_score, h->out_s + offset, (size_t)count * sizeof(float), hipMemcpyDeviceToHost, h->stream));
  HIPCHK(h, hipStreamSynchronize(h->stream));
  return APSS_OK;
}

int32_t apss_size(const apss_handle *h, int64_t *rows, int64_t *nnz) {
  if (!h) return APSS_E_INVALID;
  if (rows) *rows = h->n_rows;
  if (nnz) *nnz = h->nnz;
  return APSS_OK;
}

int32_t apss_stats_get(apss_handle *h, apss_stats *out) {
  if (!h || !out) return APSS_E_INVALID;
  h->st.rows = h->n_rows;
  h->st.nnz = h->nnz;
  h->st.tiles = h->use_coarse && h->ex_built_rows < h->idx_rows ? h->cx.n_tiles : ceil_div(h->idx_rows, h->ex.cb);
  h->st.hbm_bytes = (int64_t)h->bytes_reserved;
  h->st.downgrades = h->downgrades;
  h->st.head_terms = h->head_k ? (int64_t)h->head_terms.size() : 0;
  h->st.head_columns = (uint32_t)h->head_k;
  const int32_t caller = out->struct_size;
  if (caller < (int32_t)(2 * sizeof(int32_t)) || caller > (1 << 16))
    return fail(h, APSS_E_INVALID, "apss_stats.struct_size must be set to sizeof(apss_stats) before the call");
  const int32_t n = std::min<int32_t>(caller, (int32_t)sizeof(apss_stats));
  h->st.struct_size = n;
  std::memcpy(out, &h->st, (size_t)n);
  return APSS_OK;
}

int32_t apss_insert_dev(apss_handle *h, int64_t n, int64_t nnz, const int64_t *d_rowptr, const int32_t *d_indices,
                        const float *d_values, const int64_t *d_ext_ids) {
  APSS_TRY(enter(h));
  if (n < 0 || nnz < 0) return fail(h, APSS_E_INVALID, "negative size");
  if (n > 0 && (!d_rowptr || !d_ext_ids || (nnz > 0 && (!d_indices || !d_values))))
    return fail(h, APSS_E_INVALID, "null device pointer");
  int64_t first = 0;
  return insert_dev_impl(h, n, nnz, d_rowptr, d_indices, d_values, d_ext_ids, &first);
}

int32_t apss_insert_stored_dev(apss_handle *h, int64_t n, int64_t nnz, const int64_t *d_rowptr, const int32_t *d_indices,
                               const float *d_values, const int64_t *d_ext_ids) {
  APSS_TRY(enter(h));
  if (n < 0 || nnz < 0) return fail(h, APSS_E_INVALID, "negative size");
  if (n > 0 && (!d_rowptr || !d_ext_ids || (nnz > 0 && (!d_indices || !d_values))))
    return fail(h, APSS_E_INVALID, "null device pointer");
  int64_t first = 0;
  h->stored_rows = true;
  const int32_t rc = insert_dev_impl(h, n, nnz, d_rowptr, d_indices, d_values, d_ext_ids, &first);
  h->stored_rows = false;
  return rc;
}

int32_t apss_get_store_dev(apss_handle *h, const int64_t **d_rowptr, const int32_t **d_indices, const float **d_values, int64_t *rows,
                       int64_t *nnz) {
  if (!h) return APSS_E_INVALID;
  const bool any = h->n_rows > 0;
  if (d_rowptr) *d_rowptr = any ? h->rowptr.p : nullptr;
  if (d_indices) *d_indices = any ? h->idx.p : nullptr;
  if (d_values) *d_values = any ? h->val.p : nullptr;
  if (rows) *rows = h->n_rows;
  if (nnz) *nnz = h->nnz;
  return APSS_OK;
}

int32_t apss_query_dev(apss_handle *h, int64_t n, int64_t nnz, const int64_t *d_rowptr, const int32_t *d_indices,
                       const float *d_values, const int64_t *d_ext_ids, int64_t *n_results) {
  APSS_TRY(enter(h));
  if (n < 0 || nnz < 0) return fail(h, APSS_E_INVALID, "negative size");
  if (n > 0 && (!d_rowptr || !d_ext_ids || (nnz > 0 && (!d_indices || !d_values))))
    return fail(h, APSS_E_INVALID, "null device pointer");
  return query_dev_impl(h, n, nnz, d_rowptr, d_indices, d_values, d_ext_ids, n_results);
}

int32_t apss_insert_and_query_dev(apss_handle *h, int64_t n, int64_t nnz, const int64_t *d_rowptr,
                                  const int32_t *d_indices, const float *d_values, const int64_t *d_ext_ids,
                                  int64_t *n_results) {
  APSS_TRY(enter(h));
  if (n < 0 || nnz < 0) return fail(h, APSS_E_INVALID, "negative size");
  if (n > 0 && (!d_rowptr || !d_ext_ids || (nnz > 0 && (!d_indices || !d_values))))
    return fail(h, APSS_E_INVALID, "null device pointer");
  int64_t first = 0;
  APSS_TRY(insert_dev_impl(h, n, nnz, d_rowptr, d_indices, d_values, d_ext_ids, &first));
  const int64_t nq = h->n_rows - first;
  return probe(h, nq, h->rowptr.p + first, h->idx.p, h->val.p, h->ext.p + first, first, h->store_max_nnz, h->store_max_norm2, h->nnz,
               n_results);
}

int32_t apss_clear(apss_handle *h) {
  APSS_TRY(enter(h));
  HIPCHK(h, hipStreamSynchronize(h->stream));
  h->n_rows = 0;
  h->idx_rows = 0;
  h->nnz = 0;
  h->n_tiles = 0;
  for (apss_handle::IndexSet *s : {&h->ex, &h->cx}) { s->n_tiles = 0; s->post_used = 0; s->h_base.clear(); s->built_rows = 0; }
  h->ex_built_rows = 0;
  h->n_res = -1;
  h->res_q_ext = nullptr;
  h->last_q_rowptr = nullptr;
  h->last_q_idx = nullptr;
  h->last_q_val = nullptr;
  h->last_nq = 0;
  h->nonneg = true;
  h->q_nonneg = true;
  h->no_acc8 = h->dbgcfg.no_acc8;
  h->merge_off = false;
  h->downgrades = 0;
  h->store_max_nnz = 0;
  h->store_max_norm2 = 0.f;
  h->store_nonempty = 0;
  if (!h->head_fixed) {
    h->head_k = 0;
    h->head_terms.clear();
  }
  h->head_eval_rows = 0;
  h->head_blocked = false;
  h->head_nonempty = 0;
  return APSS_OK;
}

int32_t apss_set_head_terms(apss_handle *h, int32_t n_terms, const int32_t *terms, int32_t part, int32_t n_parts) {
  APSS_TRY(enter(h));
  if (h->n_rows != 0) return fail(h, APSS_E_STATE, "apss_set_head_terms: the handle holds vectors (set the block before the first insert or after apss_clear)");
  if (n_terms < 0 || n_terms > kHeadMaxTerms || (n_terms > 0 && !terms)) return fail(h, APSS_E_INVALID, "apss_set_head_terms: 0 .. 32768 terms");
  if (n_parts < 1 || part < 0 || part >= n_parts) return fail(h, APSS_E_INVALID, "apss_set_head_terms: part must be in [0, n_parts)");
  if (n_parts > 1 && !h->sharded)
    return fail(h, APSS_E_INVALID, "apss_set_head_terms: only a term shard multiplies a share of the block (n_parts > 1)");
  if (n_terms == 0) {
    h->head_fixed = false;
    h->head_k = 0;
    h->head_terms.clear();
    h->head_part = 0;
    h->head_parts = 1;
    return APSS_OK;
  }
  if (!h->use_coarse || !(h->cfg.theta > 0.0))
    return fail(h, APSS_E_UNSUPPORTED, "a dense-head block needs the two-pass join (theta > 0, no EXACT_ACCUM / FORCE_* flag)");
  if (h->sharded && (h->cfg.flags & APSS_FLAG_ADMISSION))
    return fail(h, APSS_E_UNSUPPORTED, "a term shard packs the block's rows from the batch row by row: not with APSS_FLAG_ADMISSION");
  if (!(h->dbgcfg.fold_w == 128 || h->dbgcfg.fold_w == 256) && !h->dbgcfg.mix) {
    h->head_fold_w = h->head_fold_user ? h->head_fold_user : 128;
    h->head_exact = 256 - h->head_fold_w;
  }
  std::vector<int32_t> pos((size_t)h->cfg.dim, -1);
  for (int32_t i = 0; i < n_terms; ++i) {
    if (terms[i] < 0 || terms[i] >= h->cfg.dim || pos[(size_t)terms[i]] >= 0)
      return fail(h, APSS_E_INVALID, "apss_set_head_terms: terms must be distinct and in [0, dim)");
    pos[(size_t)terms[i]] = head_column(i, h->head_fold_w, h->head_exact);
  }
  APSS_TRY(ensure(h, h->head_pos, (size_t)h->cfg.dim));
  HIPCHK(h, hipMemcpyAsync(h->head_pos.p, pos.data(), (size_t)h->cfg.dim * sizeof(int32_t), hipMemcpyHostToDevice, h->stream));
  HIPCHK(h, hipStreamSynchronize(h->stream));
  h->head_terms.assign(terms, terms + n_terms);
  h->head_k = head_width(n_terms, h->head_fold_w, h->head_exact, head_wants_i8(h));
  h->head_fixed = true;
  h->head_blocked = false;
  h->head_part = part;
  h->head_parts = n_parts;
  h->cx.n_tiles = 0;
  h->ex_built_rows = 0;
  return APSS_OK;
}

int32_t apss_set_head_fold(apss_handle *h, int32_t columns) {
  APSS_TRY(enter(h));
  if (columns != 0 && columns != 64 && columns != 128 && columns != 192) return fail(h, APSS_E_INVALID, "apss_set_head_fold: 0 (default: 128), 64, 128 or 192 columns");
  if (h->n_rows != 0) return fail(h, APSS_E_STATE, "apss_set_head_fold: on an empty handle (it takes effect at the next apss_set_head_terms)");
  h->head_fold_user = columns;
  return APSS_OK;
}

int32_t apss_get_head_terms(apss_handle *h, int32_t capacity, int32_t *out_terms, int32_t *n_terms) {
  if (!h || !n_terms) return APSS_E_INVALID;
  const int32_t n = h->head_k ? (int32_t)h->head_terms.size() : 0;
  *n_terms = n;
  if (out_terms)
    for (int32_t i = 0; i < std::min(n, capacity); ++i) out_terms[i] = h->head_terms[(size_t)i];
  return APSS_OK;
}

int32_t apss_set_top_k(apss_handle *h, int32_t k) {
  APSS_TRY(enter(h));
  if (k < 0 || k > APSS_TOP_K_MAX) return fail(h, APSS_E_INVALID, g_create_error = "apss_set_top_k: k must be in [0, 1024] (0: off)");
  if (k > 0 && h->sharded)
    return fail(h, APSS_E_UNSUPPORTED, g_create_error = "apss_set_top_k: a term shard reports candidates with partial scores; the group cuts behind its exchange");
  h->top_k = k;
  return APSS_OK;
}

int32_t apss_topk_get(apss_handle *h, apss_topk_info *out) {
  if (!h || !out) return APSS_E_INVALID;
  const int32_t caller = out->struct_size;
  if (caller < (int32_t)(2 * sizeof(int32_t)) || caller > (1 << 16))
    return fail(h, APSS_E_INVALID, "apss_topk_info.struct_size must be set to sizeof(apss_topk_info) before the call");
  const int32_t n = std::min<int32_t>(caller, (int32_t)sizeof(apss_topk_info));
  h->tk.struct_size = n;
  std::memcpy(out, &h->tk, (size_t)n);
  return APSS_OK;
}

int32_t apss_ext_ids_dev(apss_handle *h, const int64_t **d_store_ext, const int64_t **d_query_ext) {
  if (!h) return APSS_E_INVALID;
  if (d_store_ext) *d_store_ext = h->n_rows > 0 ? h->ext.p : nullptr;
  if (d_query_ext) *d_query_ext = h->res_q_ext;
  return APSS_OK;
}

int32_t apss_results_dev(apss_handle *h, const int32_t **d_q_row, const int32_t **d_c_slot, const float **d_score,
                         int64_t *n_results) {
  if (!h) return APSS_E_INVALID;
  if (h->n_res < 0) return fail(h, APSS_E_STATE, "no query has run on this handle");
  if (d_q_row) *d_q_row = h->out_q;
  if (d_c_slot) *d_c_slot = h->out_c;
  if (d_score) *d_score = h->out_s;
  if (n_results) *n_results = h->n_res;
  return APSS_OK;
}

int32_t apss_results_copy_dev(apss_handle *h, int64_t offset, int64_t count, int32_t *d_q_row, int32_t *d_c_slot,
                              float *d_score) {
  APSS_TRY(enter(h));
  if (h->n_res < 0) return fail(h, APSS_E_STATE, "no query has run on this handle since the last insert");
  if (offset < 0 || count < 0 || offset + count > h->n_res) return fail(h, APSS_E_INVALID, "copy range out of bounds");
  if (count == 0) return APSS_OK;
  if (d_q_row) HIPCHK(h, hipMemcpyAsync(d_q_row, h->out_q + offset, (size_t)count * sizeof(int32_t), hipMemcpyDeviceToDevice, h->stream));
  if (d_c_slot) HIPCHK(h, hipMemcpyAsync(d_c_slot, h->out_c + offset, (size_t)count * sizeof(int32_t), hipMemcpyDeviceToDevice, h->stream));
  if (d_score) HIPCHK(h, hipMemcpyAsync(d_score, h->out_s + offset, (size_t)count * sizeof(float), hipMemcpyDeviceToDevice, h->stream));
  return APSS_OK;
}

int32_t apss_partial_scores_dev(apss_handle *h, int64_t n_pairs, const int32_t *d_q_row, const int32_t *d_c_slot,
                                float *d_out_partial) {
  APSS_TRY(enter(h));
  if (n_pairs < 0) return fail(h, APSS_E_INVALID, "negative pair count");
  if (n_pairs == 0) return APSS_OK;
  if (!h->last_q_rowptr) return fail(h, APSS_E_STATE, "no query batch on this handle since the last insert");
  if (!d_q_row || !d_c_slot || !d_out_partial) return fail(h, APSS_E_INVALID, "null device pointer");
  PartialArgs a{};
  a.n_pairs = n_pairs;
  a.q_row = d_q_row;
  a.c_slot = d_c_slot;
  a.q_rowptr = h->last_q_rowptr;
  a.q_idx = h->last_q_idx;
  a.q_val = h->last_q_val;
  a.c_rowptr = h->rowptr.p;
  a.c_idx = h->idx.p;
  a.c_val = h->val.p;
  a.out = d_out_partial;
  a.nq = h->last_nq;
  a.n_rows = h->n_rows;
  for (int64_t p0 = 0; p0 < n_pairs; p0 += (1LL << 27)) {
    PartialArgs aa = a;
    aa.n_pairs = std::min<int64_t>(1LL << 27, n_pairs - p0);
    aa.q_row = d_q_row + p0;
    aa.c_slot = d_c_slot + p0;
    aa.out = d_out_partial + p0;
    hipLaunchKernelGGL(k_partial_scores, dim3((unsigned)ceil_div(aa.n_pairs * kGroup, 256)), dim3(256), 0, h->stream, aa);
    HIPCHK(h, hipGetLastError());
  }
  HIPCHK(h, hipStreamSynchronize(h->stream));
  return APSS_OK;
}

}
```

all-pairs-similarity_amd/csrc/apss_kernels.hpp:

```cpp
#pragma once
#include <hip/hip_fp16.h>
#include <hip/hip_runtime.h>
#include <stdint.h>

namespace apss {

constexpr int kWave = 64;
constexpr int kGroup = 16;
constexpr int kItemCap = 2048;
constexpr int kLongCap = 256;
constexpr int kLongLen = 64;
constexpr int kSurvCap = 1024;
constexpr int kProbeBlock = 1024;

struct alignas(8) Posting {
  uint32_t slot;
  float w;
};

template <typename T>
__device__ __forceinline__ T uniform_load(const T *p) {
  return *reinterpret_cast<const __attribute__((address_space(4))) T *>(reinterpret_cast<uintptr_t>(p));
}

constexpr int kUnmergedBit = 0x40000000;
enum Counter { kCtrResults = 0, kCtrVisits = 1, kCtrCands = 2, kCtrFlags = 3, kCtrDevVisits = 4, kCtrSnap = 5, kCtrPre = 6, kCtrOver = 7, kCtrCount = 8 };

__device__ __forceinline__ uint64_t wave_append(bool pred, unsigned long long *counter) {
  const unsigned long long mask = __ballot(pred);
  if (mask == 0) return ~0ull;
  const int lane = __lane_id();
  const int leader = __ffsll((long long)mask) - 1;
  unsigned long long base = 0;
  if (lane == leader) base = atomicAdd(counter, (unsigned long long)__popcll(mask));
  base = __shfl(base, leader);
  const unsigned long long below = mask & ((1ull << lane) - 1ull);
  return pred ? base + (unsigned long long)__popcll(below) : ~0ull;
}


struct IngestArgs {
  int64_t n;
  int64_t nnz;
  const int64_t *rowptr;
  const int32_t *idx;
  const float *val;
  int32_t dim, term_lo, term_hi;
  uint32_t flags;
  float theta, index_threshold;
  const int32_t *head_pos;
  int64_t *row_keep;
  int64_t *row_cnt;
  float *row_inv;
  float *row_sub;
  unsigned int *flags_out;
};

template <int G>
__global__ void k_ingest_count(IngestArgs a) {
  __shared__ unsigned sh[4];
  if (threadIdx.x < 4) sh[threadIdx.x] = 0;
  __syncthreads();
  const int gl = threadIdx.x % G;
  const int64_t rows_per_sweep = (int64_t)gridDim.x * (blockDim.x / G);
  for (int64_t row = ((int64_t)blockIdx.x * blockDim.x + threadIdx.x) / G; row - threadIdx.x / G < a.n; row += rows_per_sweep) {
  int64_t b = 0, e = 0;
  if (row < a.n) {
    b = a.rowptr[row];
    e = a.rowptr[row + 1];
  }
  unsigned bad = 0;
  if (b < 0 || e < b || e > a.nnz || (row == 0 && b != 0)) {
    bad |= 1;
    b = e = 0;
  }
  const bool normalise = (a.flags & 4u) != 0;
  float sumsq = 0.f, sum = 0.f, sub = 0.f, full = 0.f;
  int cnt = 0;
  auto account = [&](const float v, const int32_t t) {
    sum += v;
    const bool keep_v = !(a.flags & 1u) || v > a.index_threshold;
    if (keep_v) full += v * v;
    const bool keep = keep_v && t >= a.term_lo && t < a.term_hi;
    if (keep) {
      cnt++;
      if (!a.head_pos || a.head_pos[t] < 0) sub += v * v;
      if (v < 0.f) bad |= 4;
    }
  };
  for (int64_t k = b + gl; k < e; k += G) {
    const float v = a.val[k];
    const int32_t t = a.idx[k];
    if (!(t >= 0 && t < a.dim) || (k > b && a.idx[k - 1] >= t)) bad |= 1;
    if (!isfinite(v)) bad |= 2;
    sumsq += v * v;
    if (!normalise) account(v, t);
  }
  float inv = 1.0f;
  if (normalise) {
    for (int o = G / 2; o; o >>= 1) sumsq += __shfl_xor(sumsq, o, G);
    inv = sumsq > 0.f ? 1.0f / sqrtf(sumsq) : 0.f;
    for (int64_t k = b + gl; k < e; k += G) account(a.val[k] * inv, a.idx[k]);
  }
  for (int o = G / 2; o; o >>= 1) {
    sum += __shfl_xor(sum, o, G);
    full += __shfl_xor(full, o, G);
    sub += __shfl_xor(sub, o, G);
    cnt += __shfl_xor(cnt, o, G);
    bad |= __shfl_xor(bad, o, G);
  }
  if (gl == 0 && row < a.n) {
    const bool admit = !(a.flags & 2u) || sum >= a.theta;
    a.row_keep[row] = admit ? 1 : 0;
    a.row_cnt[row] = admit ? cnt : 0;
    a.row_inv[row] = inv;
    a.row_sub[row] = full > 0.f ? fminf(1.0f, sqrtf(sub / full)) * 0.999999f : 0.f;
    if (bad) atomicOr(&sh[0], bad);
    if (admit) {
      atomicMax(&sh[1], (unsigned)cnt);
      atomicMax(&sh[2], __float_as_uint(full));
      if (cnt > 0) atomicAdd(&sh[3], 1u);
    }
  }
  }
  __syncthreads();
  if (threadIdx.x == 0) {
    if (sh[0]) atomicOr(a.flags_out, sh[0]);
    if (sh[1]) atomicMax(a.flags_out + 1, sh[1]);
    if (sh[2]) atomicMax(a.flags_out + 2, sh[2]);
    if (sh[3]) atomicAdd(a.flags_out + 3, sh[3]);
  }
}

struct IngestWriteArgs {
  IngestArgs in;
  const int64_t *row_dst;
  const int64_t *nnz_dst;
  int64_t dst_row0, dst_nnz0;
  int64_t *o_rowptr;
  int32_t *o_idx;
  float *o_val;
  int64_t *o_ext;
  float *o_sub;
  uint32_t *o_erow;
  const int64_t *ext;
};

__global__ void k_ingest_write(IngestWriteArgs w) {
  const IngestArgs &a = w.in;
  const int64_t row = ((int64_t)blockIdx.x * blockDim.x + threadIdx.x) / kGroup;
  const int gl = threadIdx.x % kGroup;
  if (row >= a.n) return;
  if (!a.row_keep[row]) return;
  const int64_t b = a.rowptr[row], e = a.rowptr[row + 1];
  const float inv = a.row_inv[row];
  const int64_t dr = w.dst_row0 + (w.row_dst ? w.row_dst[row] : row);
  int64_t out = w.dst_nnz0 + w.nnz_dst[row];
  for (int64_t k0 = b; k0 < e; k0 += kGroup) {
    const int64_t k = k0 + gl;
    bool keep = false;
    float v = 0.f;
    int32_t t = 0;
    if (k < e) {
      v = a.val[k] * inv;
      t = a.idx[k];
      keep = (!(a.flags & 1u) || v > a.index_threshold) && t >= a.term_lo && t < a.term_hi;
    }
    const unsigned long long m = __ballot(keep);
    const int lane = __lane_id();
    const int gbase = lane & ~(kGroup - 1);
    const unsigned gm = (unsigned)((m >> gbase) & 0xffffu);
    if (keep) {
      const int64_t o = out + __popc(gm & ((1u << gl) - 1u));
      w.o_idx[o] = t;
      w.o_val[o] = v;
      if (w.o_erow) w.o_erow[o] = (uint32_t)dr;
    }
    out += __popc(gm);
  }
  if (gl == 0) {
    w.o_rowptr[dr + 1] = w.dst_nnz0 + w.nnz_dst[row] + a.row_cnt[row];
    w.o_ext[dr] = w.ext[row];
    if (w.o_sub) w.o_sub[dr] = a.row_sub[row];
  }
}

__global__ __launch_bounds__(1024) void k_scan_i64(const int64_t *in, int64_t *out, int64_t n) {
  __shared__ int64_t part[1024];
  const int tid = threadIdx.x;
  const int64_t per = (n + 1023) / 1024;
  const int64_t b = (int64_t)tid * per, e = b + per < n ? b + per : n;
  int64_t s = 0;
  for (int64_t i = b; i < e; ++i) s += in[i];
  part[tid] = s;
  __syncthreads();
  for (int o = 1; o < 1024; o <<= 1) {
    int64_t v = tid >= o ? part[tid - o] : 0;
    __syncthreads();
    part[tid] += v;
    __syncthreads();
  }
  int64_t run = part[tid] - s;
  for (int64_t i = b; i < e; ++i) {
    const int64_t v = in[i];
    out[i] = run;
    run += v;
  }
  if (tid == 1023) out[n] = part[1023];
}

constexpr int kScanBlock = 4096;
template <typename T>
__device__ __forceinline__ T block_excl_scan_1024(T v, T *wave_tot , T *total) {
  const int tid = threadIdx.x, ln = tid % kWave, wv = tid / kWave;
  T x = v;
#pragma unroll
  for (int o = 1; o < kWave; o <<= 1) {
    const T y = __shfl_up(x, o);
    if (ln >= o) x += y;
  }
  if (ln == kWave - 1) wave_tot[wv] = x;
  __syncthreads();
  if (tid == 0) {
    T run = 0;
    for (int w = 0; w < 16; ++w) {
      const T t = wave_tot[w];
      wave_tot[w] = run;
      run += t;
    }
    wave_tot[16] = run;
  }
  __syncthreads();
  *total = wave_tot[16];
  return wave_tot[wv] + x - v;
}
__global__ __launch_bounds__(1024) void k_scan_sums(const int64_t *in, int64_t *sums, int64_t n) {
  __shared__ int64_t wave_tot[17];
  const int64_t base = (int64_t)blockIdx.x * kScanBlock + (int64_t)threadIdx.x * 4;
  int64_t s = 0;
#pragma unroll
  for (int k = 0; k < 4; ++k) s += base + k < n ? in[base + k] : 0;
  int64_t total;
  (void)block_excl_scan_1024(s, wave_tot, &total);
  if (threadIdx.x == 0) sums[blockIdx.x] = total;
}
__global__ __launch_bounds__(1024) void k_scan_apply(const int64_t *in, const int64_t *block_off, int64_t *out, int64_t n, int64_t n_blocks) {
  __shared__ int64_t wave_tot[17];
  const int64_t base = (int64_t)blockIdx.x * kScanBlock + (int64_t)threadIdx.x * 4;
  int64_t v[4], s = 0;
#pragma unroll
  for (int k = 0; k < 4; ++k) {
    v[k] = base + k < n ? in[base + k] : 0;
    s += v[k];
  }
  int64_t total;
  int64_t run = block_off[blockIdx.x] + block_excl_scan_1024(s, wave_tot, &total);
#pragma unroll
  for (int k = 0; k < 4; ++k) {
    if (base + k < n) out[base + k] = run;
    run += v[k];
  }
  if (blockIdx.x == 0 && threadIdx.x == 0) out[n] = block_off[n_blocks];
}

constexpr int kSegAlign = 16;
constexpr int kSegAlignC = 32;

__device__ __forceinline__ uint32_t pack_coarse(uint32_t slot, float w) {
  return (slot & 0xffffu) | (max((uint32_t)__half_as_ushort(__float2half_rn(w)), 1u) << 16);
}

__device__ __forceinline__ uint32_t pack_coarse_wide(uint32_t slot, float w) {
  return (slot << 15) | max((uint32_t)__half_as_ushort(__float2half_rn(w)) & 0x7fffu, 1u);
}

struct BuildArgs {
  const int64_t *rowptr;
  const int32_t *idx;
  const float *val;
  int64_t row0, row1;
  int32_t cb;
  int32_t dim;
  uint2 *tile_seg;
  int64_t seg_stride;
  const int64_t *tile_post_base;
  Posting *post;
  uint32_t *post_c;
  int32_t coarse;
  int32_t coarse_shift;
  int32_t seg_align;
  int32_t coarse_wide;
  const uint32_t *erow;
  const float *row_scale;
  int32_t range_terms;
  const int64_t *ent_base;
  const uint32_t *run_cut;
  int32_t term_lo, term_hi;
  int32_t sub_shift, n_sub;
  unsigned long long *sub_cnt;
  const int64_t *sub_base;
  uint2 *o_ent;
};

__global__ void k_tile_hist(BuildArgs a) {
  const int64_t row = a.row0 + ((int64_t)blockIdx.x * blockDim.x + threadIdx.x) / kWave;
  const int lane = threadIdx.x % kWave;
  if (row >= a.row1) return;
  uint2 *sg = a.tile_seg + (row / a.cb) * a.seg_stride;
  const int64_t b = a.rowptr[row], e = a.rowptr[row + 1];
  for (int64_t k = b + lane; k < e; k += kWave) {
    const int32_t t = a.idx[k];
    if ((uint32_t)t < (uint32_t)a.dim) atomicAdd(&sg[t].y, 1u);
  }
}

__global__ __launch_bounds__(1024) void k_tile_scan_part(const uint2 *tile_seg, int64_t seg_stride, int32_t dim, int64_t tile0,
                                                         int32_t n_blk, uint32_t align, uint32_t *part, uint32_t *max_len,
                                                         unsigned long long *chunk_w, uint32_t count_long) {
  __shared__ uint32_t wave_tot[17];
  const int64_t tile = tile0 + blockIdx.x / n_blk;
  const int32_t blk = (int32_t)(blockIdx.x % n_blk);
  const uint2 *sg = tile_seg + tile * seg_stride;
  const int tid = threadIdx.x;
  const int32_t i0 = blk * kScanBlock + tid * 4;
  uint32_t s = 0, longest = 0, n_long = 0;
  unsigned long long cw = 0;
#pragma unroll
  for (int k = 0; k < 4; ++k) {
    const uint32_t len = i0 + k < dim ? sg[i0 + k].y : 0u;
    s += (len + align - 1) / align * align;
    longest = max(longest, len);
    n_long += len > 256u ? 1u : 0u;
    cw += len <= 256u ? (unsigned long long)len * ((len + 15u) / 16u) : 0ull;
  }
  uint32_t total;
  (void)block_excl_scan_1024<uint32_t>(s, wave_tot, &total);
  if (tid == 0) part[blockIdx.x] = total;
  __shared__ uint32_t sh_long[2];
  __shared__ unsigned long long sh_cw;
  if (tid == 0) {
    sh_long[0] = sh_long[1] = 0u;
    sh_cw = 0ull;
  }
  __syncthreads();
  for (int o = kWave / 2; o; o >>= 1) {
    longest = max(longest, (uint32_t)__shfl_xor((int)longest, o));
    n_long += (uint32_t)__shfl_xor((int)n_long, o);
  }
  for (int o = kWave / 2; o; o >>= 1) cw += __shfl_xor(cw, o);
  if ((tid % kWave) == 0) {
    if (longest) atomicMax(&sh_long[0], longest);
    if (n_long) atomicAdd(&sh_long[1], n_long);
    if (cw) atomicAdd(&sh_cw, cw);
  }
  __syncthreads();
  if (tid == 0) {
    if (max_len && sh_long[0]) {
      atomicMax(max_len, sh_long[0]);
      if (sh_long[1] && count_long) atomicAdd(max_len + 1, sh_long[1]);
    }
    if (chunk_w && sh_cw) atomicAdd(chunk_w, sh_cw);
  }
}

__global__ __launch_bounds__(1024) void k_tile_scan_place(uint2 *tile_seg, int64_t seg_stride, int32_t dim, int64_t tile0, int32_t n_blk,
                                                          uint32_t align, uint32_t keep_len, const uint32_t *part, int64_t *tile_total) {
  __shared__ uint32_t wave_tot[17];
  __shared__ uint32_t before;
  const int64_t tile = tile0 + blockIdx.x / n_blk;
  const int32_t blk = (int32_t)(blockIdx.x % n_blk);
  uint2 *sg = tile_seg + tile * seg_stride;
  const int tid = threadIdx.x;
  uint32_t mine = 0u;
  for (int32_t j = tid; j < blk; j += 1024) mine += part[(blockIdx.x / n_blk) * n_blk + j];
  uint32_t tot_before;
  (void)block_excl_scan_1024<uint32_t>(mine, wave_tot, &tot_before);
  if (tid == 0) before = tot_before;
  __syncthreads();
  const uint32_t carry = before;
  const int32_t i0 = blk * kScanBlock + tid * 4;
  uint32_t len[4], s = 0;
#pragma unroll
  for (int k = 0; k < 4; ++k) {
    len[k] = i0 + k < dim ? sg[i0 + k].y : 0u;
    s += (len[k] + align - 1) / align * align;
  }
  uint32_t total;
  uint32_t run = carry + block_excl_scan_1024<uint32_t>(s, wave_tot, &total);
#pragma unroll
  for (int k = 0; k < 4; ++k) {
    if (i0 + k < dim) sg[i0 + k] = make_uint2(run, keep_len ? len[k] : 0u);
    run += (len[k] + align - 1) / align * align;
  }
  if (blk == n_blk - 1 && tid == 0) tile_total[tile] = (int64_t)carry + (int64_t)total;
}

__global__ void k_tile_scatter(BuildArgs a) {
  const int64_t row = a.row0 + ((int64_t)blockIdx.x * blockDim.x + threadIdx.x) / kWave;
  const int lane = threadIdx.x % kWave;
  if (row >= a.row1) return;
  const int64_t tile = row / a.cb;
  uint2 *sg = a.tile_seg + tile * a.seg_stride;
  const int64_t pbase = a.tile_post_base[tile];
  const uint32_t local = (uint32_t)(row - tile * a.cb);
  const int64_t b = a.rowptr[row], e = a.rowptr[row + 1];
  for (int64_t k = b + lane; k < e; k += kWave) {
    const int32_t t = a.idx[k];
    if ((uint32_t)t >= (uint32_t)a.dim) continue;
    const unsigned long long old = atomicAdd(reinterpret_cast<unsigned long long *>(&sg[t]), 1ull << 32);
    const uint32_t pos = (uint32_t)old + (uint32_t)(old >> 32);
    if (a.coarse) {
      const float sc = a.row_scale ? a.row_scale[row] : 1.0f;
      const float wv_ = sc > 0.f ? a.val[k] / sc : a.val[k];
      a.post_c[pbase + pos] = a.coarse_wide ? pack_coarse_wide(local, wv_) : pack_coarse(local << a.coarse_shift, wv_);
    } else {
      Posting p;
      p.slot = local;
      p.w = a.val[k];
      a.post[pbase + pos] = p;
    }
  }
}

struct ShiftArgs {
  const uint2 *seg_old;
  uint2 *seg_new;
  const uint32_t *old_c;
  const Posting *old_x;
  uint32_t *new_c;
  Posting *new_x;
  int32_t dim;
};
__global__ void k_tile_shift(ShiftArgs a) {
  const int64_t t = ((int64_t)blockIdx.x * blockDim.x + threadIdx.x) / kGroup;
  const int gl = threadIdx.x % kGroup;
  if (t >= a.dim) return;
  const uint2 o = a.seg_old[t];
  const uint32_t n0 = a.seg_new[t].x;
  if (a.old_c) {
    for (uint32_t i = gl; i < o.y; i += kGroup) a.new_c[n0 + i] = a.old_c[o.x + i];
  } else {
    for (uint32_t i = gl; i < o.y; i += kGroup) a.new_x[n0 + i] = a.old_x[o.x + i];
  }
  if (gl == 0) a.seg_new[t].y = o.y;
}

constexpr int kBuildRange = 16384;
constexpr int kBuildMaxRanges = 16;

__global__ __launch_bounds__(1024) void k_tile_hist_lds(BuildArgs a, int64_t tile0, int32_t n_ranges) {
  __shared__ uint32_t cnt[kBuildRange];
  const int tid = threadIdx.x;
  const int64_t tile = tile0 + blockIdx.x / n_ranges;
  const int32_t rt = a.range_terms ? a.range_terms : kBuildRange;
  const int32_t lo = (int32_t)(blockIdx.x % n_ranges) * rt;
  const uint32_t span = (uint32_t)(min(a.dim, lo + rt) - lo);
  for (int i = tid; i < rt; i += 1024) cnt[i] = 0u;
  __syncthreads();
  const int64_t rA = tile * a.cb, rB = min(a.row1, rA + (int64_t)a.cb);
  const int64_t eA = a.ent_base ? a.ent_base[blockIdx.x] : a.rowptr[rA], eB = a.ent_base ? a.ent_base[blockIdx.x + 1] : a.rowptr[rB];
  for (int64_t k = eA + tid; k < eB; k += 4096) {
    int32_t t[4];
#pragma unroll
    for (int j = 0; j < 4; ++j) t[j] = k + 1024 * j < eB ? a.idx[k + 1024 * j] : -1;
#pragma unroll
    for (int j = 0; j < 4; ++j)
      if ((uint32_t)(t[j] - lo) < span) atomicAdd(&cnt[t[j] - lo], 1u);
  }
  __syncthreads();
  uint2 *sg = a.tile_seg + tile * a.seg_stride + lo;
  for (uint32_t i = tid; i < span; i += 1024) sg[i] = make_uint2(0u, cnt[i]);
}

__global__ __launch_bounds__(1024) void k_tile_scatter_lds(BuildArgs a, int64_t tile0, int32_t n_ranges) {
  __shared__ uint32_t cur[kBuildRange];
  const int tid = threadIdx.x;
  const int64_t tile = tile0 + blockIdx.x / n_ranges;
  const int32_t rt = a.range_terms ? a.range_terms : kBuildRange;
  const int32_t lo = (int32_t)(blockIdx.x % n_ranges) * rt;
  const uint32_t span = (uint32_t)(min(a.dim, lo + rt) - lo);
  const uint2 *sg = a.tile_seg + tile * a.seg_stride + lo;
  for (uint32_t i = tid; i < span; i += 1024) cur[i] = sg[i].x;
  __syncthreads();
  const int64_t pbase = a.tile_post_base[tile];
  const int64_t rA = tile * a.cb, rB = min(a.row1, rA + (int64_t)a.cb);
  const int64_t eA = a.ent_base ? a.ent_base[blockIdx.x] : a.rowptr[rA], eB = a.ent_base ? a.ent_base[blockIdx.x + 1] : a.rowptr[rB];
// ... 1980 lines not shown
```

Baseline: 1003 billion.

## Fuse plain ingest into one kernel that also emits run cuts and df sample

When no transform (prune, admission, normalize, sharding) is needed, ingest now runs a single kernel. That kernel validates rows, copies idx/val/erow straight to their final positions, and writes rowptr and ext. This replaces the count kernel, the two scans, the host round trip and the write kernel. The same kernel also precomputes the per-row run cut offsets used by the run-based tile build, so build can reuse them instead of launching k_row_cuts, and it samples document frequencies for the head policy. The cost is a more complex kernel, extra cut storage, and a dependence on the predicted tile and range parameters matching those used at build time.

```diff
diff --git a/all-pairs-similarity_amd/csrc/apss_hip.hip b/all-pairs-similarity_amd/csrc/apss_hip.hip
--- a/all-pairs-similarity_amd/csrc/apss_hip.hip
+++ b/all-pairs-similarity_amd/csrc/apss_hip.hip
@@ -68,6 +68,7 @@
   bool no_merge_prune = false;
   int merge_u = 0;
   int merge_single = 0;
+  bool no_fused_ingest = false;
 };
 
 DebugCfg parse_debug_env() {
@@ -123,6 +124,7 @@
     else if (key == "merge_u") d.merge_u = (int)val;
     else if (key == "no_merge_prune") d.no_merge_prune = val != 0;
     else if (key == "merge_single") d.merge_single = (int)val;
+    else if (key == "no_fused_ingest") d.no_fused_ingest = val != 0;
     else if (key == "relayout_fail") {}
     else if (!key.empty()) fprintf(stderr, "[apss] unknown APSS_DEBUG token '%s' ignored\n", key.c_str());
   }
@@ -196,6 +198,11 @@
   DevBuf<float> bk_val;
   DevBuf<uint32_t> run_cut;
   DevBuf<uint2> run_ent;
+  DevBuf<uint32_t> ing_cut;
+  int64_t cut_lo = 0, cut_hi = 0;
+  int32_t cut_cb = 0, cut_rt = 0, cut_ranges = 0;
+  std::vector<uint32_t> df_host;
+  int64_t df_rows = -1, df_stride = 0;
   DevBuf<uint2> app_seg;
   DevBuf<char> app_post;
   DevBuf<int32_t> vq_first, vrow_q;
@@ -337,6 +344,115 @@
 int32_t head_fit_scale(apss_handle *h, double norm2, unsigned char *W, int64_t packed_bytes);
 inline void head_pack_rendering(const apss_handle *h, HeadPackArgs &p);
 
+bool ingest_wants_cuts(const apss_handle *h, int64_t dst_row0, int64_t n, int64_t nnz, int32_t *cb, int32_t *rt, int32_t *n_ranges);
+bool head_policy_due(const apss_handle *h, int64_t n_rows);
+
+int32_t take_ingest_flags(apss_handle *h, const unsigned int *flags_host, bool to_store) {
+  if (flags_host[0] & 1u)
+    return fail(h, APSS_E_INVALID, "malformed vector: indices must be strictly increasing and in [0, dim) "
+                                   "(SparseVector.scala:75; vectorDim mismatch is the require of CommonUtils.scala:99)");
+  if (flags_host[0] & 2u) return fail(h, APSS_E_INVALID, "non-finite value in a vector");
+  if (to_store) h->nonneg = h->nonneg && !(flags_host[0] & 4u);
+  else h->q_nonneg = !(flags_host[0] & 4u);
+  float norm2;
+  std::memcpy(&norm2, &flags_host[2], sizeof(float));
+  if (to_store) {
+    h->store_max_nnz = std::max<int64_t>(h->store_max_nnz, flags_host[1]);
+    h->store_max_norm2 = std::max(h->store_max_norm2, norm2);
+    h->store_nonempty += flags_host[3];
+    h->last_batch_nonempty = flags_host[3];
+  } else {
+    h->q_max_nnz = flags_host[1];
+    h->q_max_norm2 = norm2;
+  }
+  return APSS_OK;
+}
+
+int32_t ingest_plain(apss_handle *h, int64_t n, int64_t nnz, const int64_t *d_rowptr, const int32_t *d_idx, const float *d_val,
+                     const int64_t *d_ext, bool to_store, int64_t *n_out, int64_t *nnz_out) {
+  APSS_TRY(ensure(h, h->flagword, 4));
+  const int64_t dst_row0 = to_store ? h->n_rows : 0, dst_nnz0 = to_store ? h->nnz : 0;
+  DevBuf<int64_t> &o_rowptr = to_store ? h->rowptr : h->q_rowptr;
+  DevBuf<int64_t> &o_ext = to_store ? h->ext : h->q_ext;
+  DevBuf<int32_t> &o_idx = to_store ? h->idx : h->q_idx;
+  DevBuf<float> &o_val = to_store ? h->val : h->q_val;
+  APSS_TRY(ensure(h, o_rowptr, (size_t)(dst_row0 + n + 1), (size_t)(to_store ? dst_row0 + 1 : 0)));
+  APSS_TRY(ensure(h, o_ext, (size_t)(dst_row0 + n), (size_t)dst_row0));
+  APSS_TRY(ensure(h, o_idx, (size_t)(dst_nnz0 + nnz), (size_t)dst_nnz0));
+  APSS_TRY(ensure(h, o_val, (size_t)(dst_nnz0 + nnz), (size_t)dst_nnz0));
+  if (to_store) APSS_TRY(ensure(h, h->erow, (size_t)(dst_nnz0 + nnz), (size_t)dst_nnz0));
+  HIPCHK(h, hipMemsetAsync(h->flagword.p, 0, 4 * sizeof(unsigned int), h->stream));
+  if (dst_row0 == 0) HIPCHK(h, hipMemsetAsync(o_rowptr.p, 0, sizeof(int64_t), h->stream));
+
+  IngestPlainArgs p{};
+  IngestArgs &a = p.w.in;
+  a.n = n;
+  a.nnz = nnz;
+  a.rowptr = d_rowptr;
+  a.idx = d_idx;
+  a.val = d_val;
+  a.dim = h->cfg.dim;
+  a.flags_out = h->flagword.p;
+  p.w.dst_row0 = dst_row0;
+  p.w.dst_nnz0 = dst_nnz0;
+  p.w.o_rowptr = o_rowptr.p;
+  p.w.o_idx = o_idx.p;
+  p.w.o_val = o_val.p;
+  p.w.o_ext = o_ext.p;
+  p.w.o_erow = to_store ? h->erow.p : nullptr;
+  p.w.ext = d_ext;
+  int32_t cut_cb = 0, cut_rt = 0, cut_ranges = 0;
+  const bool cuts = to_store && ingest_wants_cuts(h, dst_row0, n, nnz, &cut_cb, &cut_rt, &cut_ranges);
+  bool cuts_extend = false;
+  if (cuts) {
+    cuts_extend = h->cut_hi > h->cut_lo && h->cut_hi == dst_row0 && h->cut_cb == cut_cb && h->cut_rt == cut_rt && h->cut_ranges == cut_ranges;
+    if (!cuts_extend) h->cut_lo = h->cut_hi = 0;
+    const size_t cw = (size_t)cut_ranges + 1;
+    APSS_TRY(ensure(h, h->ing_cut, (size_t)(dst_row0 + n) * cw, cuts_extend ? (size_t)dst_row0 * cw : 0));
+    p.cut = h->ing_cut.p;
+    p.n_ranges = cut_ranges;
+    p.range_terms = cut_rt;
+    p.cb = cut_cb;
+  }
+  const bool sample = to_store && dst_row0 == 0 && head_policy_due(h, n);
+  const int32_t dim = h->cfg.dim;
+  if (to_store) h->df_rows = -1;
+  if (sample) {
+    APSS_TRY(ensure(h, h->df, (size_t)dim));
+    HIPCHK(h, hipMemsetAsync(h->df.p, 0, (size_t)dim * sizeof(uint32_t), h->stream));
+    p.df = h->df.p;
+    p.df_stride = std::max<int64_t>(1, n / 65536);
+    h->df_host.resize((size_t)dim);
+  }
+  const int threads = 256;
+  const int64_t blocks = ceil_div(n * kGroup, threads);
+  hipLaunchKernelGGL(k_ingest_plain, dim3((unsigned)std::min<int64_t>(blocks, 4096)), dim3(threads), 0, h->stream, p);
+  HIPCHK(h, hipGetLastError());
+  unsigned int flags_stack[4] = {0, 0, 0, 0};
+  unsigned int *flags_host = h->pin ? reinterpret_cast<unsigned int *>(h->pin + kPinBytes) : flags_stack;
+  HIPCHK(h, hipMemcpyAsync(flags_host, h->flagword.p, 4 * sizeof(unsigned int), hipMemcpyDeviceToHost, h->stream));
+  if (sample) HIPCHK(h, hipMemcpyAsync(h->df_host.data(), h->df.p, (size_t)dim * sizeof(uint32_t), hipMemcpyDeviceToHost, h->stream));
+  HIPCHK(h, hipStreamSynchronize(h->stream));
+  if (h->dbgcfg.diag)
+    fprintf(stderr, "[apss diag] ingest fused: %lld %s rows at %lld, cuts %s, df sample %s\n", (long long)n, to_store ? "store" : "query",
+            (long long)dst_row0, cuts ? (cuts_extend ? "appended" : "written") : "none", sample ? "taken" : "none");
+  APSS_TRY(take_ingest_flags(h, flags_host, to_store));
+  if (cuts) {
+    if (!cuts_extend) h->cut_lo = dst_row0;
+    h->cut_hi = dst_row0 + n;
+    h->cut_cb = cut_cb;
+    h->cut_rt = cut_rt;
+    h->cut_ranges = cut_ranges;
+  }
+  if (sample) {
+    h->df_rows = n;
+    h->df_stride = p.df_stride;
+  }
+  *n_out = n;
+  *nnz_out = nnz;
+  return APSS_OK;
+}
+
 int32_t ingest(apss_handle *h, int64_t n, int64_t nnz, const int64_t *d_rowptr, const int32_t *d_idx,
                const float *d_val, const int64_t *d_ext, bool to_store, int64_t *n_out, int64_t *nnz_out) {
   *n_out = 0;
@@ -344,6 +460,10 @@
   if (n == 0) return APSS_OK;
   const uint32_t in_flags = h->stored_rows ? h->cfg.flags & ~(APSS_FLAG_VALUE_PRUNE | APSS_FLAG_ADMISSION | APSS_FLAG_NORMALIZE) : h->cfg.flags;
   const bool transform = h->sharded || (in_flags & (APSS_FLAG_VALUE_PRUNE | APSS_FLAG_ADMISSION | APSS_FLAG_NORMALIZE));
+  if (!transform && !h->dbgcfg.no_fused_ingest) return ingest_plain(h, n, nnz, d_rowptr, d_idx, d_val, d_ext, to_store, n_out, nnz_out);
+  if (h->dbgcfg.diag)
+    fprintf(stderr, "[apss diag] ingest unfused: %lld %s rows at %lld (%s)\n", (long long)n, to_store ? "store" : "query",
+            (long long)(to_store ? h->n_rows : 0), transform ? "transform" : "no_fused_ingest");
   APSS_TRY(ensure(h, h->s_keep, (size_t)n + 1));
   APSS_TRY(ensure(h, h->s_cnt, (size_t)n + 1));
   APSS_TRY(ensure(h, h->s_inv, (size_t)n));
@@ -390,23 +510,7 @@
   }
   HIPCHK(h, hipMemcpyAsync(flags_host, h->flagword.p, 4 * sizeof(unsigned int), hipMemcpyDeviceToHost, h->stream));
   HIPCHK(h, hipStreamSynchronize(h->stream));
-  if (flags_host[0] & 1u)
-    return fail(h, APSS_E_INVALID, "malformed vector: indices must be strictly increasing and in [0, dim) "
-                                   "(SparseVector.scala:75; vectorDim mismatch is the require of CommonUtils.scala:99)");
-  if (flags_host[0] & 2u) return fail(h, APSS_E_INVALID, "non-finite value in a vector");
-  if (to_store) h->nonneg = h->nonneg && !(flags_host[0] & 4u);
-  else h->q_nonneg = !(flags_host[0] & 4u);
-  float norm2;
-  std::memcpy(&norm2, &flags_host[2], sizeof(float));
-  if (to_store) {
-    h->store_max_nnz = std::max<int64_t>(h->store_max_nnz, flags_host[1]);
-    h->store_max_norm2 = std::max(h->store_max_norm2, norm2);
-    h->store_nonempty += flags_host[3];
-    h->last_batch_nonempty = flags_host[3];
-  } else {
-    h->q_max_nnz = flags_host[1];
-    h->q_max_norm2 = norm2;
-  }
+  APSS_TRY(take_ingest_flags(h, flags_host, to_store));
 
   DevBuf<int64_t> &o_rowptr = to_store ? h->rowptr : h->q_rowptr;
   DevBuf<int64_t> &o_ext = to_store ? h->ext : h->q_ext;
@@ -592,6 +696,33 @@
   else hipLaunchKernelGGL((k_tile_runs<SCATTER, 32>), grid, dim3(1024), lds, stream, b, tile0, n_ranges);
 }
 
+struct BuildForm {
+  int32_t n_ranges, bucket_rt, run_rt;
+  bool bucket_build, lds_build, run_build;
+  double mean_run;
+};
+BuildForm build_form(const apss_handle *h, int64_t cb, int64_t tile0, int64_t n_tiles, int64_t rows, int64_t build_nnz, int64_t max_nnz) {
+  int32_t n_ranges = (int32_t)ceil_div(h->cfg.dim, kBuildRange);
+  int32_t bucket_rt = h->dbgcfg.bucket_range > 0 ? h->dbgcfg.bucket_range : 8192;
+  while (ceil_div(h->cfg.dim, bucket_rt) > kBucketMaxRanges && bucket_rt < kBuildRange) bucket_rt *= 2;
+  const bool bucket_build = n_ranges > kBuildMaxRanges && ceil_div(h->cfg.dim, bucket_rt) <= kBucketMaxRanges && !h->dbgcfg.build_atomic &&
+                            !h->dbgcfg.no_bucket && tile0 == 0 && n_tiles * n_ranges >= 48 && build_nnz > 0 && build_nnz <= (1LL << 32) &&
+                            n_tiles * (int64_t)kBucketSlices < (1LL << 31);
+  if (bucket_build) n_ranges = (int32_t)ceil_div(h->cfg.dim, bucket_rt);
+  const bool lds_build = bucket_build || (n_ranges <= kBuildMaxRanges && !h->dbgcfg.build_atomic &&
+                                          ((n_tiles - tile0) * n_ranges >= 48 || h->dbgcfg.build_lds));
+  const double mean_row = rows > 0 ? (double)build_nnz / (double)rows : 0.0;
+  int32_t run_rt = h->dbgcfg.run_range > 0 ? std::min(h->dbgcfg.run_range, kBuildRange) : kRunRange;
+  const int64_t t_lo = h->cfg.term_lo, t_hi = h->cfg.term_hi;
+  const int64_t run_active = std::max<int64_t>(1, ceil_div(t_hi, run_rt) - t_lo / run_rt);
+  const double mean_run = mean_row / (double)run_active;
+  const bool run_build = lds_build && !bucket_build && !h->dbgcfg.build_stream && std::max<int64_t>(max_nnz, 1) * cb < (1LL << 31) &&
+                         ceil_div(h->cfg.dim, run_rt) <= 64 &&
+                         (h->dbgcfg.build_runs || (n_ranges >= 2 && mean_row >= kRunMinMeanRow));
+  if (run_build) n_ranges = (int32_t)ceil_div(h->cfg.dim, run_rt);
+  return BuildForm{n_ranges, bucket_rt, run_rt, bucket_build, lds_build, run_build, mean_run};
+}
+
 int32_t build_tiles(apss_handle *h, apss_handle::IndexSet &ix, int64_t row0) {
   const int64_t cb = ix.cb;
   int64_t tile0 = row0 / cb;
@@ -630,27 +761,13 @@
   if (ix.h_base.empty()) ix.h_base.push_back(0);
   ix.h_base.resize((size_t)tile0 + 1);
   const int64_t r0 = tile0 * cb;
-  int32_t n_ranges = (int32_t)ceil_div(h->cfg.dim, kBuildRange);
   const int64_t build_nnz = h->head_k ? h->tv.nnz : h->nnz;
-  int32_t bucket_rt = h->dbgcfg.bucket_range > 0 ? h->dbgcfg.bucket_range : 8192;
-  while (ceil_div(h->cfg.dim, bucket_rt) > kBucketMaxRanges && bucket_rt < kBuildRange) bucket_rt *= 2;
-  const bool bucket_build = n_ranges > kBuildMaxRanges && ceil_div(h->cfg.dim, bucket_rt) <= kBucketMaxRanges && !h->dbgcfg.build_atomic &&
-                            !h->dbgcfg.no_bucket && tile0 == 0 && n_tiles * n_ranges >= 48 && build_nnz > 0 && build_nnz <= (1LL << 32) &&
-                            n_tiles * (int64_t)kBucketSlices < (1LL << 31);
-  if (bucket_build) n_ranges = (int32_t)ceil_div(h->cfg.dim, bucket_rt);
-  const bool lds_build = bucket_build || (n_ranges <= kBuildMaxRanges && !h->dbgcfg.build_atomic &&
-                                          ((n_tiles - tile0) * n_ranges >= 48 || h->dbgcfg.build_lds));
+  const BuildForm form = build_form(h, cb, tile0, n_tiles, h->idx_rows, build_nnz, h->store_max_nnz);
+  const int32_t n_ranges = form.n_ranges, bucket_rt = form.bucket_rt, run_rt = form.run_rt;
+  const bool bucket_build = form.bucket_build, lds_build = form.lds_build, run_build = form.run_build;
+  const double mean_run = form.mean_run;
   if (!lds_build)
     HIPCHK(h, hipMemsetAsync(ix.seg.p + tile0 * stride, 0, (size_t)((n_tiles - tile0) * stride) * sizeof(uint2), h->stream));
-  const double mean_row = h->idx_rows > 0 ? (double)build_nnz / (double)h->idx_rows : 0.0;
-  int32_t run_rt = h->dbgcfg.run_range > 0 ? std::min(h->dbgcfg.run_range, kBuildRange) : kRunRange;
-  const int64_t t_lo = h->cfg.term_lo, t_hi = h->cfg.term_hi;
-  const int64_t run_active = std::max<int64_t>(1, ceil_div(t_hi, run_rt) - t_lo / run_rt);
-  const double mean_run = mean_row / (double)run_active;
-  const bool run_build = lds_build && !bucket_build && !h->dbgcfg.build_stream && std::max<int64_t>(h->store_max_nnz, 1) * cb < (1LL << 31) &&
-                         ceil_div(h->cfg.dim, run_rt) <= 64 &&
-                         (h->dbgcfg.build_runs || (n_ranges >= 2 && mean_row >= kRunMinMeanRow));
-  if (run_build) n_ranges = (int32_t)ceil_div(h->cfg.dim, run_rt);
   BuildArgs b{};
   fill_build_args(h, ix, b, scaled);
   b.row0 = r0;
@@ -669,10 +786,15 @@
             (long long)tile0, (long long)n_tiles, bucket_build ? "bucketed" : (run_build ? "runs" : (lds_build ? "stream" : "atomic")), (int)n_ranges,
             run_build ? run_rt : (bucket_build ? bucket_rt : kBuildRange), run_build ? run_lanes : 0, mean_run);
   if (h->dbgcfg.build_trace && run_build) fprintf(stderr, "[apss]   scatter through sub-ranges of %d terms\n", (int)run_sub);
+  const bool cuts_on_hand = run_build && !h->head_k && h->cut_cb == (int32_t)cb && h->cut_rt == run_rt && h->cut_ranges == n_ranges &&
+                            h->cut_lo <= r0 && h->cut_hi >= h->idx_rows && h->cut_hi > h->cut_lo;
+  if (h->dbgcfg.diag && run_build)
+    fprintf(stderr, "[apss diag] build %s rows [%lld, %lld): cuts %s\n", ix.coarse ? "coarse" : "exact", (long long)r0, (long long)h->idx_rows,
+            cuts_on_hand ? "reused" : "computed");
   if (run_build) {
-    APSS_TRY(ensure(h, h->run_cut, (size_t)((h->idx_rows - r0) * (n_ranges + 1))));
+    if (!cuts_on_hand) APSS_TRY(ensure(h, h->run_cut, (size_t)((h->idx_rows - r0) * (n_ranges + 1))));
     b.range_terms = run_rt;
-    b.run_cut = h->run_cut.p;
+    b.run_cut = cuts_on_hand ? h->ing_cut.p + r0 * (n_ranges + 1) : h->run_cut.p;
     if (run_sub) {
       APSS_TRY(ensure(h, h->bk_cnt, (size_t)n_bk + 2));
       APSS_TRY(ensure(h, h->bk_base, (size_t)n_bk + 2));
@@ -756,8 +878,9 @@
   const size_t run_lds = (size_t)run_rt * sizeof(uint32_t);
   if (bucket_build) {}
   else if (run_build) {
-    hipLaunchKernelGGL(k_row_cuts, dim3((unsigned)ceil_div((h->idx_rows - r0) * kGroup, threads)), dim3(threads), 0, h->stream, b, n_ranges,
-                       h->run_cut.p);
+    if (!cuts_on_hand)
+      hipLaunchKernelGGL(k_row_cuts, dim3((unsigned)ceil_div((h->idx_rows - r0) * kGroup, threads)), dim3(threads), 0, h->stream, b, n_ranges,
+                         h->run_cut.p);
     launch_tile_runs<kRunHist>(run_lanes, lds_grid, run_lds, h->stream, b, tile0, n_ranges);
     if (run_sub) {
       APSS_TRY(scan_i64(h, reinterpret_cast<const int64_t *>(h->bk_cnt.p), h->bk_base.p, n_bk));
@@ -832,6 +955,32 @@
   return 0.0;
 }
 
+int32_t pick_cx_tile(const apss_handle *h, int64_t rows, int64_t nnz, int64_t max_nnz, float max_norm2) {
+  const double seg32 = 32768.0 * ((double)nnz / (double)rows) / (double)h->cfg.dim;
+  int32_t cb = seg32 < 16.0 && !h->sharded && !h->head_k ? 65536 : 32768;
+  if (cb == 65536 && seg32 < 8.0 && h->nonneg && !h->dbgcfg.no_acc8 && !h->no_acc8 && max_nnz <= 512 &&
+      acc8_scale((double)max_norm2 * 1.0001 + 1e-6, (double)max_nnz, h->cfg.theta) > 0)
+    cb = 131072;
+  if ((h->sharded || h->head_k) && !(h->head_k && h->head_longseg) && !h->dbgcfg.no_acc8 && !h->no_acc8 &&
+      acc8_scale((double)max_norm2 * 1.0001 + 1e-6, (double)max_nnz, h->cfg.theta) > 0)
+    cb = 65536;
+  return cb;
+}
+
+bool ingest_wants_cuts(const apss_handle *h, int64_t dst_row0, int64_t n, int64_t nnz, int32_t *cb, int32_t *rt, int32_t *n_ranges) {
+  if (h->head_k) return false;
+  const int64_t rows = dst_row0 + n, entries = h->nnz + nnz;
+  const apss_handle::IndexSet &ix = h->use_coarse ? h->cx : h->ex;
+  *cb = ix.cb;
+  if (h->use_coarse && ix.n_tiles == 0 && h->cfg.tile_rows == 0 && !h->dbgcfg.cx_tile)
+    *cb = pick_cx_tile(h, rows, entries, h->store_max_nnz, h->store_max_norm2);
+  if (*cb <= 0) return false;
+  const BuildForm form = build_form(h, *cb, std::min(h->idx_rows, dst_row0) / *cb, ceil_div(rows, *cb), rows, entries, h->store_max_nnz);
+  *rt = form.run_rt;
+  *n_ranges = form.n_ranges;
+  return form.run_build && form.n_ranges <= 2 * kGroup - 1;
+}
+
 constexpr int64_t kTailMaxRows = 1024;
 constexpr int64_t kTailMaxBatch = 64;
 constexpr int64_t kTailMaxPairs = 1 << 22;
@@ -850,6 +999,9 @@
 inline bool head_allowed(const apss_handle *h) {
   return h->use_coarse && (!h->sharded || h->head_fixed) && (h->cfg.head_terms >= 0 || h->head_fixed) && h->cfg.theta > 0.0 &&
          !h->head_blocked && h->nonneg;
+}
+bool head_policy_due(const apss_handle *h, int64_t n_rows) {
+  return head_allowed(h) && !h->head_fixed && n_rows >= std::max<int64_t>(h->cfg.head_terms > 0 ? 1 : kHeadMinRows, 2 * h->head_eval_rows);
 }
 
 inline bool head_wants_i8(const apss_handle *h) {
@@ -1062,14 +1214,22 @@
   h->head_eval_rows = n;
   const int64_t stride = std::max<int64_t>(1, n / 65536);
   const int64_t sampled = ceil_div(n, stride);
-  APSS_TRY(ensure(h, h->df, (size_t)dim));
-  HIPCHK(h, hipMemsetAsync(h->df.p, 0, (size_t)dim * sizeof(uint32_t), h->stream));
-  hipLaunchKernelGGL(k_df_sample, dim3((unsigned)ceil_div(sampled * kWave, 256)), dim3(256), 0, h->stream,
-                     (const int64_t *)h->rowptr.p, (const int32_t *)h->idx.p, n, stride, h->df.p);
-  HIPCHK(h, hipGetLastError());
-  std::vector<uint32_t> df((size_t)dim);
-  HIPCHK(h, hipMemcpyAsync(df.data(), h->df.p, (size_t)dim * sizeof(uint32_t), hipMemcpyDeviceToHost, h->stream));
-  HIPCHK(h, hipStreamSynchronize(h->stream));
+  std::vector<uint32_t> df;
+  const bool delivered = h->df_rows == n && h->df_stride == stride && h->df_host.size() == (size_t)dim;
+  if (delivered) {
+    df.swap(h->df_host);
+  } else {
+    APSS_TRY(ensure(h, h->df, (size_t)dim));
+    HIPCHK(h, hipMemsetAsync(h->df.p, 0, (size_t)dim * sizeof(uint32_t), h->stream));
+    hipLaunchKernelGGL(k_df_sample, dim3((unsigned)ceil_div(sampled * kWave, 256)), dim3(256), 0, h->stream,
+                       (const int64_t *)h->rowptr.p, (const int32_t *)h->idx.p, n, stride, h->df.p);
+    HIPCHK(h, hipGetLastError());
+    df.resize((size_t)dim);
+    HIPCHK(h, hipMemcpyAsync(df.data(), h->df.p, (size_t)dim * sizeof(uint32_t), hipMemcpyDeviceToHost, h->stream));
+    HIPCHK(h, hipStreamSynchronize(h->stream));
+  }
+  h->df_rows = -1;
+  if (h->dbgcfg.diag) fprintf(stderr, "[apss diag] head policy: df sample of %lld rows %s\n", (long long)n, delivered ? "reused" : "computed");
   std::vector<int32_t> order((size_t)dim);
   for (int32_t t = 0; t < dim; ++t) order[(size_t)t] = t;
   const size_t top = (size_t)std::min<int32_t>(dim, kHeadMaxTerms);
@@ -1162,7 +1322,7 @@
   row0 = std::min(row0, h->idx_rows);
   h->idx_rows = h->n_rows;
   if (head_allowed(h)) {
-    if (!h->head_fixed && h->n_rows >= std::max<int64_t>(h->cfg.head_terms > 0 ? 1 : kHeadMinRows, 2 * h->head_eval_rows)) {
+    if (head_policy_due(h, h->n_rows)) {
       bool changed = false;
       APSS_TRY(choose_head(h, &changed));
       if (changed) {
@@ -1189,14 +1349,7 @@
   }
   if (h->use_coarse) {
     if (h->cx.n_tiles == 0 && h->cfg.tile_rows == 0 && !h->dbgcfg.cx_tile && h->idx_rows > 0) {
-      const double seg32 = 32768.0 * ((double)h->nnz / (double)h->n_rows) / (double)h->cfg.dim;
-      h->cx.cb = seg32 < 16.0 && !h->sharded && !h->head_k ? 65536 : 32768;
-      if (h->cx.cb == 65536 && seg32 < 8.0 && h->nonneg && !h->dbgcfg.no_acc8 && !h->no_acc8 && h->store_max_nnz <= 512 &&
-          acc8_scale((double)h->store_max_norm2 * 1.0001 + 1e-6, (double)h->store_max_nnz, h->cfg.theta) > 0)
-        h->cx.cb = 131072;
-      if ((h->sharded || h->head_k) && !(h->head_k && h->head_longseg) && !h->dbgcfg.no_acc8 && !h->no_acc8 &&
-          acc8_scale((double)h->store_max_norm2 * 1.0001 + 1e-6, (double)h->store_max_nnz, h->cfg.theta) > 0)
-        h->cx.cb = 65536;
+      h->cx.cb = pick_cx_tile(h, h->n_rows, h->nnz, h->store_max_nnz, h->store_max_norm2);
     }
     APSS_TRY(build_tiles(h, h->cx, row0));
     h->st.build_ms += h->cx.build_ms;
@@ -2367,6 +2520,12 @@
 
 int32_t query_dev_impl(apss_handle *h, int64_t n, int64_t nnz, const int64_t *d_rowptr, const int32_t *d_idx,
                        const float *d_val, const int64_t *d_ext, int64_t *n_results) {
+  h->n_res = -1;
+  h->res_q_ext = nullptr;
+  h->last_q_rowptr = nullptr;
+  h->last_q_idx = nullptr;
+  h->last_q_val = nullptr;
+  h->last_nq = 0;
   int64_t kept_rows = 0, kept_nnz = 0;
   APSS_TRY(ingest(h, n, nnz, d_rowptr, d_idx, d_val, d_ext, false, &kept_rows, &kept_nnz));
   if (h->head_k && !h->sharded && kept_rows > 0) APSS_TRY(pack_query_head(h, h->q_rowptr.p, h->q_idx.p, h->q_val.p, kept_rows));
@@ -2485,7 +2644,7 @@
   release(h->head_pos); release(h->W);
   for (apss_handle::TailView *v : {&h->tv, &h->qtv}) { release(v->rowptr); release(v->idx); release(v->val); release(v->erow); }
   release(h->tv_cnt); release(h->tv_off); release(h->tv_sum); release(h->q_W); release(h->df); release(h->dedup_tab);
-  release(h->head_ctr); release(h->uq_q); release(h->uq_c); release(h->uq_s); release(h->pack); release(h->chain_ctr); release(h->app_seg); release(h->app_post); release(h->bk_cnt); release(h->bk_base); release(h->bk_idx); release(h->bk_erow); release(h->bk_val); release(h->run_cut); release(h->run_ent);
+  release(h->head_ctr); release(h->uq_q); release(h->uq_c); release(h->uq_s); release(h->pack); release(h->chain_ctr); release(h->app_seg); release(h->app_post); release(h->bk_cnt); release(h->bk_base); release(h->bk_idx); release(h->bk_erow); release(h->bk_val); release(h->run_cut); release(h->run_ent); release(h->ing_cut);
   topk_release(h->topk);
   if (h->pin) (void)hipHostFree(h->pin);
   if (h->ev0) (void)hipEventDestroy(h->ev0);
@@ -2701,6 +2860,8 @@
   h->head_eval_rows = 0;
   h->head_blocked = false;
   h->head_nonempty = 0;
+  h->cut_lo = h->cut_hi = 0;
+  h->df_rows = -1;
   return APSS_OK;
 }
 
diff --git a/all-pairs-similarity_amd/csrc/apss_kernels.hpp b/all-pairs-similarity_amd/csrc/apss_kernels.hpp
--- a/all-pairs-similarity_amd/csrc/apss_kernels.hpp
+++ b/all-pairs-similarity_amd/csrc/apss_kernels.hpp
@@ -80,11 +80,12 @@
   auto account = [&](const float v, const int32_t t) {
     sum += v;
     const bool keep_v = !(a.flags & 1u) || v > a.index_threshold;
-    if (keep_v) full += v * v;
+    const float sq = __fmul_rn(v, v);
+    if (keep_v) full += sq;
     const bool keep = keep_v && t >= a.term_lo && t < a.term_hi;
     if (keep) {
       cnt++;
-      if (!a.head_pos || a.head_pos[t] < 0) sub += v * v;
+      if (!a.head_pos || a.head_pos[t] < 0) sub += sq;
       if (v < 0.f) bad |= 4;
     }
   };
@@ -182,6 +183,125 @@
     w.o_rowptr[dr + 1] = w.dst_nnz0 + w.nnz_dst[row] + a.row_cnt[row];
     w.o_ext[dr] = w.ext[row];
     if (w.o_sub) w.o_sub[dr] = a.row_sub[row];
+  }
+}
+
+struct IngestPlainArgs {
+  IngestWriteArgs w;
+  uint32_t *cut;
+  int32_t n_ranges;
+  int32_t range_terms;
+  int32_t cb;
+  uint32_t *df;
+  int64_t df_stride;
+};
+
+__global__ void k_ingest_plain(IngestPlainArgs p) {
+  const IngestWriteArgs &w = p.w;
+  const IngestArgs &a = w.in;
+  constexpr int G = kGroup;
+  __shared__ unsigned sh[4];
+  if (threadIdx.x < 4) sh[threadIdx.x] = 0;
+  __syncthreads();
+  const int gl = threadIdx.x % G;
+  const int gshift = __lane_id() & ~(G - 1);
+  const int64_t rows_per_sweep = (int64_t)gridDim.x * (blockDim.x / G);
+  const uint32_t rt = (uint32_t)p.range_terms;
+  int64_t row = ((int64_t)blockIdx.x * blockDim.x + threadIdx.x) / G;
+  int64_t b_next = 0, e_next = 0;
+  if (row < a.n) {
+    b_next = a.rowptr[row];
+    e_next = a.rowptr[row + 1];
+  }
+  for (; row < a.n; row += rows_per_sweep) {
+    int64_t b = b_next, e = e_next;
+    if (row + rows_per_sweep < a.n) {
+      b_next = a.rowptr[row + rows_per_sweep];
+      e_next = a.rowptr[row + rows_per_sweep + 1];
+    }
+    unsigned bad = 0;
+    const bool extents_ok = !(b < 0 || e < b || e > a.nnz || (row == 0 && b != 0));
+    if (!extents_ok) {
+      bad |= 1;
+      b = e = 0;
+    }
+    const int64_t dr = w.dst_row0 + row;
+    const int64_t out = w.dst_nnz0 + b;
+    const bool sampled = p.df && (uint32_t)dr % (uint32_t)p.df_stride == 0;
+    float full = 0.f;
+    uint32_t below0 = 0, below1 = 0;
+    int32_t t_prev = -1;
+    int32_t tA = 0, tB = 0, tA_next = 0, tB_next = 0;
+    float vA = 0.f, vB = 0.f, vA_next = 0.f, vB_next = 0.f;
+    auto load = [&](const int64_t k0, int32_t &t0, float &v0, int32_t &t1, float &v1) {
+      const int64_t k = k0 + gl;
+      t0 = k < e ? a.idx[k] : 0;
+      v0 = k < e ? a.val[k] : 0.f;
+      t1 = k + G < e ? a.idx[k + G] : 0;
+      v1 = k + G < e ? a.val[k + G] : 0.f;
+    };
+    if (b < e) load(b, tA_next, vA_next, tB_next, vB_next);
+    for (int64_t k0 = b; k0 < e; k0 += 2 * G) {
+      const int64_t kA = k0 + gl, kB = kA + G;
+      const bool inA = kA < e, inB = kB < e;
+      tA = tA_next, vA = vA_next, tB = tB_next, vB = vB_next;
+      if (k0 + 2 * G < e) load(k0 + 2 * G, tA_next, vA_next, tB_next, vB_next);
+      auto chunk = [&](const int64_t k, const bool in, const int32_t t, const float v) {
+        int32_t tp = __shfl_up(t, 1, G);
+        if (gl == 0) tp = t_prev;
+        t_prev = __shfl(t, G - 1, G);
+        const bool in_dim = in && (uint32_t)t < (uint32_t)a.dim;
+        if (in) {
+          if (!in_dim || tp >= t) bad |= 1;
+          if (!isfinite(v)) bad |= 2;
+          if (v < 0.f) bad |= 4;
+          full += __fmul_rn(v, v);
+          const int64_t o = out + (k - b);
+          w.o_idx[o] = t;
+          w.o_val[o] = v;
+          if (w.o_erow) w.o_erow[o] = (uint32_t)dr;
+          if (sampled && in_dim) atomicAdd(&p.df[t], 1u);
+        }
+        if (p.cut) {
+          for (int32_t j = 1; j <= p.n_ranges; ++j) {
+            const uint32_t c = (uint32_t)__popc((unsigned)((__ballot(in_dim && (uint32_t)t < (uint32_t)j * rt) >> gshift) & 0xffffu));
+            if (j == gl) below0 += c;
+            if (j == gl + G) below1 += c;
+          }
+        }
+      };
+      chunk(kA, inA, tA, vA);
+      if (k0 + G < e) chunk(kB, inB, tB, vB);
+    }
+    for (int o = G / 2; o; o >>= 1) {
+      full += __shfl_xor(full, o, G);
+      bad |= __shfl_xor(bad, o, G);
+    }
+    if (extents_ok && p.cut) {
+      const int64_t tr = (int64_t)((uint32_t)dr / (uint32_t)p.cb) * p.cb;
+      const int64_t tb = tr >= w.dst_row0 ? w.dst_nnz0 + a.rowptr[tr - w.dst_row0] : w.o_rowptr[tr];
+      uint32_t *c = p.cut + dr * (p.n_ranges + 1);
+      const uint32_t first = (uint32_t)(out - tb);
+      if (gl <= p.n_ranges) c[gl] = first + below0;
+      if (gl + G <= p.n_ranges) c[gl + G] = first + below1;
+    }
+    if (gl == 0) {
+      if (extents_ok) {
+        w.o_rowptr[dr + 1] = w.dst_nnz0 + e;
+        w.o_ext[dr] = w.ext[row];
+      }
+      if (bad) atomicOr(&sh[0], bad);
+      atomicMax(&sh[1], (unsigned)(e - b));
+      atomicMax(&sh[2], __float_as_uint(full));
+      if (e > b) atomicAdd(&sh[3], 1u);
+    }
+  }
+  __syncthreads();
+  if (threadIdx.x == 0) {
+    if (sh[0]) atomicOr(a.flags_out, sh[0]);
+    if (sh[1]) atomicMax(a.flags_out + 1, sh[1]);
+    if (sh[2]) atomicMax(a.flags_out + 2, sh[2]);
+    if (sh[3]) atomicAdd(a.flags_out + 3, sh[3]);
   }
 }
 
```

New measurement: 1021 billion, median of 6. +1.8%, better.
